# robertknight/ocrs

Measured on AMD Instinct MI355X. Metric: pages/sec end-to-end (1024x1024), higher is better.
Workload: dtype f32

## Files before the change

include/ocrs_amd.h:

```cpp
#ifndef OCRS_AMD_H
#define OCRS_AMD_H

#include <stddef.h>
#include <stdint.h>

#if defined(__GNUC__)
#define OCRS_API __attribute__((visibility("default")))
#else
#define OCRS_API
#endif

#ifdef __cplusplus
extern "C" {
#endif

typedef enum ocrs_status {
    OCRS_OK = 0,
    OCRS_ERR_INVALID_ARGUMENT = 1,
    OCRS_ERR_MODEL_NOT_LOADED = 2,
    OCRS_ERR_MODEL_DIMS = 3,
    OCRS_ERR_RUN_FAILED = 4,
    OCRS_ERR_WRONG_OUTPUT = 5,
    OCRS_ERR_IMAGE_SOURCE = 6,
    OCRS_ERR_DEVICE = 7,
    OCRS_ERR_IO = 8,
    OCRS_ERR_CAPACITY = 9
} ocrs_status;

OCRS_API const char* ocrs_last_error(void);

#define OCRS_ABI_VERSION 6u
OCRS_API uint32_t ocrs_abi_version(void);

OCRS_API void ocrs_buffer_free(void* p);

OCRS_API ocrs_status ocrs_device_count(int* n);
OCRS_API ocrs_status ocrs_set_device(int device);
OCRS_API ocrs_status ocrs_get_device(int* device);

OCRS_API ocrs_status ocrs_ctc_beam_search(const float* logp, int t, int c, uint32_t width, int impl, uint32_t** labels,
                                          uint32_t** positions, size_t* n);
OCRS_API ocrs_status ocrs_ctc_beam_search_scored(const float* logp, int t, int c, uint32_t width, int impl, uint32_t** labels,
                                                 uint32_t** positions, size_t* n, double* score, float** step_logp);

OCRS_API ocrs_status ocrs_gru_tile_plan(const int32_t* lengths_desc, size_t n_lines, int hidden, int32_t* n_clusters, int32_t* waves,
                                        int16_t* tiles);

OCRS_API ocrs_status ocrs_coalescer_selftest(int n_threads, int requests_per_thread, int max_active, int max_pages,
                                             long window_us, int fail_every, uint64_t out[5]);

OCRS_API ocrs_status ocrs_set_option(const char* name, long value);
OCRS_API ocrs_status ocrs_option_name(int index, const char** name);

OCRS_API ocrs_status ocrs_device_pool_stats(int device, uint64_t out[12]);
OCRS_API ocrs_status ocrs_device_pool_configure(int device, uint64_t device_cached_cap_bytes, uint64_t pinned_cached_cap_bytes);
OCRS_API ocrs_status ocrs_device_pool_trim(int device);

typedef enum { OCRS_ISOLATION_AUTO = 0, OCRS_ISOLATION_NONE = 1 } ocrs_isolation;
OCRS_API ocrs_status ocrs_device_set_isolation(int device, ocrs_isolation policy);
OCRS_API ocrs_status ocrs_device_isolation(int device, int out[3]);

typedef struct ocrs_model ocrs_model;

OCRS_API ocrs_status ocrs_model_load_file(const char* path, ocrs_model** out);
OCRS_API ocrs_status ocrs_model_load_bytes(const void* data, size_t len, ocrs_model** out);
OCRS_API ocrs_status ocrs_model_load_file_on_device(const char* path, int device, ocrs_model** out);
OCRS_API ocrs_status ocrs_model_load_bytes_on_device(const void* data, size_t len, int device, ocrs_model** out);
OCRS_API ocrs_status ocrs_model_device(const ocrs_model* m, int* device);

typedef int (*ocrs_model_run_fn)(void* user, const float* input, const int64_t in_shape[4], float** output,
                                 int64_t out_shape[4], int* out_ndim);
OCRS_API ocrs_status ocrs_model_from_callback(const int64_t input_shape[4],
                                     ocrs_model_run_fn run, void* user, ocrs_model** out);

OCRS_API ocrs_status ocrs_model_input_shape(const ocrs_model* m, int64_t dims[4], uint8_t is_fixed[4]);

typedef struct ocrs_run_options {
    int timing;
} ocrs_run_options;

OCRS_API ocrs_status ocrs_model_run(const ocrs_model* m, const float* input, const int64_t in_shape[4],
                           const ocrs_run_options* opts, float** output, int64_t out_shape[4], int* out_ndim);

OCRS_API ocrs_status ocrs_model_flops(const ocrs_model* m, const int64_t in_shape[4], double* flops);

OCRS_API void ocrs_model_free(ocrs_model* m);

typedef struct ocrs_engine ocrs_engine;
typedef struct ocrs_page ocrs_page;

typedef enum ocrs_numerics { OCRS_NUMERICS_EXACT = 0, OCRS_NUMERICS_RELAXED = 1, OCRS_NUMERICS_REDUCED = 2 } ocrs_numerics;

typedef enum ocrs_decode_method {
    OCRS_DECODE_GREEDY = 0,
    OCRS_DECODE_BEAM_SEARCH = 1
} ocrs_decode_method;

typedef struct ocrs_engine_params {
    const ocrs_model* detection_model;
    const ocrs_model* recognition_model;
    int debug;
    ocrs_decode_method decode_method;
    uint32_t beam_width;
    const char* alphabet;
    const char* allowed_chars;
    ocrs_numerics numerics;
    int coalesce;
    int coalesce_pages;
    int coalesce_window_us;
    int layout_threads;
    int64_t rec_max_pixels;
} ocrs_engine_params;

OCRS_API ocrs_status ocrs_engine_new(const ocrs_engine_params* params, ocrs_engine** out);
OCRS_API void ocrs_engine_free(ocrs_engine* e);
OCRS_API ocrs_status ocrs_engine_device(const ocrs_engine* e, int* device);
OCRS_API ocrs_status ocrs_engine_set_option(ocrs_engine* e, const char* name, long value);
OCRS_API ocrs_status ocrs_engine_get_option(const ocrs_engine* e, const char* name, long* value);

typedef enum ocrs_dim_order { OCRS_HWC = 0, OCRS_CHW = 1 } ocrs_dim_order;
typedef enum ocrs_pixel_type { OCRS_U8 = 0, OCRS_F32 = 1 } ocrs_pixel_type;

OCRS_API ocrs_status ocrs_image_source_check_bytes(size_t len, uint32_t width, uint32_t height, uint32_t* channels);

OCRS_API ocrs_status ocrs_engine_prepare_input(const ocrs_engine* e, const void* pixels, ocrs_pixel_type type,
                                      ocrs_dim_order order, int height, int width, int channels,
                                      ocrs_page** out);
OCRS_API ocrs_status ocrs_engine_prepare_input_batch(const ocrs_engine* e, const void* const* pixels, size_t n,
                                                     ocrs_pixel_type type, ocrs_dim_order order, int height, int width,
// ... 244 lines not shown
```

ocrs_amd/_lib.py:

```python
import ctypes as C
import os

_HERE = os.path.dirname(os.path.abspath(__file__))
LIB_PATH = os.environ.get("OCRS_AMD_LIB") or os.path.join(_HERE, "libocrs_amd.so")

OCRS_OK = 0
STATUS_NAMES = {
    0: "OK", 1: "INVALID_ARGUMENT", 2: "MODEL_NOT_LOADED", 3: "MODEL_DIMS", 4: "RUN_FAILED", 5: "WRONG_OUTPUT",
    6: "IMAGE_SOURCE", 7: "DEVICE", 8: "IO", 9: "CAPACITY",
}

RUN_FN = C.CFUNCTYPE(C.c_int, C.c_void_p, C.POINTER(C.c_float), C.POINTER(C.c_int64), C.POINTER(C.POINTER(C.c_float)),
                     C.POINTER(C.c_int64), C.POINTER(C.c_int))


class EngineParams(C.Structure):
    _fields_ = [("detection_model", C.c_void_p), ("recognition_model", C.c_void_p), ("debug", C.c_int),
                ("decode_method", C.c_int), ("beam_width", C.c_uint32), ("alphabet", C.c_char_p),
                ("allowed_chars", C.c_char_p), ("numerics", C.c_int), ("coalesce", C.c_int), ("coalesce_pages", C.c_int),
                ("coalesce_window_us", C.c_int), ("layout_threads", C.c_int), ("rec_max_pixels", C.c_int64)]


class GroupParams(C.Structure):
    _fields_ = [("detection_model", C.c_void_p), ("detection_model_len", C.c_size_t), ("recognition_model", C.c_void_p),
                ("recognition_model_len", C.c_size_t), ("devices", C.POINTER(C.c_int)), ("n_devices", C.c_size_t),
                ("debug", C.c_int), ("decode_method", C.c_int), ("beam_width", C.c_uint32), ("alphabet", C.c_char_p),
                ("allowed_chars", C.c_char_p), ("gather", C.c_int), ("numerics", C.c_int), ("coalesce", C.c_int),
                ("coalesce_pages", C.c_int), ("coalesce_window_us", C.c_int), ("layout_threads", C.c_int), ("rec_max_pixels", C.c_int64),
                ("min_block", C.c_int), ("shared_block", C.c_int)]


class RunOptions(C.Structure):
    _fields_ = [("timing", C.c_int)]


class TextCharC(C.Structure):
    _fields_ = [("ch", C.c_uint32), ("top", C.c_int32), ("left", C.c_int32), ("bottom", C.c_int32),
                ("right", C.c_int32)]


class OcrsError(RuntimeError):
    def __init__(self, status, message):
        super().__init__(message)
        self.status = status
        self.status_name = STATUS_NAMES.get(status, str(status))


DECLARED_SYMBOLS = [
    "ocrs_last_error", "ocrs_buffer_free", "ocrs_device_count", "ocrs_set_device", "ocrs_set_option", "ocrs_ctc_beam_search", "ocrs_model_load_file",
    "ocrs_model_load_bytes", "ocrs_model_from_callback", "ocrs_model_input_shape", "ocrs_model_run",
    "ocrs_model_flops", "ocrs_model_free", "ocrs_engine_new", "ocrs_engine_free", "ocrs_image_source_check_bytes",
    "ocrs_engine_prepare_input", "ocrs_engine_prepare_input_device", "ocrs_page_free", "ocrs_page_dims",
    "ocrs_page_image", "ocrs_engine_detect_words", "ocrs_engine_detect_words_batch",
    "ocrs_engine_detect_text_pixels", "ocrs_engine_detection_threshold", "ocrs_engine_find_text_lines",
    "ocrs_engine_find_text_lines_batch",
    "ocrs_engine_recognize_text", "ocrs_engine_recognize_text_batch", "ocrs_engine_recognize_tokens",
    "ocrs_engine_prepare_recognition_input", "ocrs_text_item_rotated_rect", "ocrs_rotated_rect_corners", "ocrs_engine_get_text", "ocrs_device_malloc", "ocrs_device_free",
    "ocrs_device_upload", "ocrs_device_synchronize", "ocrs_device_measure_peaks", "ocrs_engine_enable_timing", "ocrs_stage_count",
    "ocrs_stage_name", "ocrs_engine_stage_times", "ocrs_kernel_class_count", "ocrs_kernel_class_name",
    "ocrs_engine_kernel_stats", "ocrs_engine_set_kernel_timing_mask", "ocrs_gru_tile_plan", "ocrs_host_malloc", "ocrs_host_free", "ocrs_engine_prepare_input_batch",
    "ocrs_get_device", "ocrs_model_load_file_on_device", "ocrs_model_load_bytes_on_device", "ocrs_model_device", "ocrs_engine_device",
    "ocrs_engine_group_new", "ocrs_engine_group_free", "ocrs_engine_group_size", "ocrs_engine_group_member", "ocrs_group_deal",
    "ocrs_group_prepare_input_batch", "ocrs_group_prepare_input_device_batch", "ocrs_group_detect_words_batch",
    "ocrs_group_recognize_text_batch", "ocrs_group_gather", "ocrs_group_final_gather", "ocrs_group_worker_threads", "ocrs_group_last_gather", "ocrs_device_malloc_on", "ocrs_engine_coalesce_stats", "ocrs_coalescer_selftest", "ocrs_engine_kernel_mfma_flops", "ocrs_engine_prepare_input_jpeg", "ocrs_jpeg_decode_rgb", "ocrs_jpeg_info", "ocrs_jpeg_coefficients",
    "ocrs_group_member_stats", "ocrs_numa_parse_cpulist", "ocrs_numa_bind_selftest", "ocrs_engine_recognize_logits", "ocrs_engine_set_option", "ocrs_engine_get_option", "ocrs_option_name", "ocrs_device_pool_stats", "ocrs_device_pool_configure", "ocrs_device_pool_trim",
    "ocrs_device_set_isolation", "ocrs_device_isolation", "ocrs_group_set_replay", "ocrs_abi_version",
    "ocrs_engine_recognize_text_scored", "ocrs_engine_recognize_text_batch_scored", "ocrs_ctc_beam_search_scored",
    "ocrs_engine_run_recognition_ops",
    "ocrs_engine_detect_words_scored", "ocrs_engine_detect_words_batch_scored", "ocrs_group_detect_words_batch_scored",
    "ocrs_engine_find_text_lines_indexed", "ocrs_engine_find_text_lines_batch_indexed",
    "ocrs_detection_tile_plan", "ocrs_engine_detect_words_tiled", "ocrs_engine_detect_words_batch_tiled",
    "ocrs_engine_detect_text_pixels_tiled", "ocrs_group_detect_words_batch_tiled",
    "ocrs_line_frame", "ocrs_line_char_boxes", "ocrs_engine_prepare_recognition_input_rectified",
    "ocrs_engine_recognize_text_rectified", "ocrs_engine_recognize_text_batch_rectified",
    "ocrs_group_recognize_text_batch_rectified", "ocrs_engine_recognize_tokens_rectified",
    "ocrs_engine_rotate_page", "ocrs_engine_rotate_pages", "ocrs_unrotate_rects", "ocrs_unrotate_chars",
    "ocrs_orientation_vote", "ocrs_engine_detect_orientation", "ocrs_engine_page_from_grey",
    "ocrs_engine_resize_page", "ocrs_engine_resize_pages", "ocrs_work_size", "ocrs_rescale_rects",
    "ocrs_engine_detect_words_at", "ocrs_engine_detect_words_batch_at",
    "ocrs_normalize_params_default", "ocrs_normalize_params_check", "ocrs_engine_normalize_page", "ocrs_engine_normalize_pages",
]

ABI_VERSION = 6
TILE_OVERLAP_DEFAULT = 100
RESAMPLE_FILTERS = {"auto": 0, "bilinear": 1, "area": 2}
POLARITIES = {"auto": 0, "keep": 1, "invert": 2}


class NormalizeParams(C.Structure):
    _fields_ = [("tile", C.c_int32), ("polarity", C.c_int32), ("flatten", C.c_int32), ("levels", C.c_int32)]


class NormalizeInfo(C.Structure):
    _fields_ = [("dark", C.c_int32), ("white", C.c_int32), ("lo", C.c_int32), ("hi", C.c_int32), ("vote", C.c_int64),
                ("counted", C.c_uint64)]

    def as_dict(self):
        return {"dark": int(self.dark), "vote": int(self.vote), "white": int(self.white), "lo": int(self.lo), "hi": int(self.hi),
                "counted": int(self.counted)}

_lib = None


def lib():
    global _lib
    if _lib is None:
        if not os.path.exists(LIB_PATH):
            raise OcrsError(7, "libocrs_amd.so is not built: run `python -m ocrs_amd.build` "
                               "(there is no CPU fallback for the HIP engine)")
        L = C.CDLL(LIB_PATH)
        L.ocrs_abi_version.restype = C.c_uint32
        if L.ocrs_abi_version() != ABI_VERSION:
            raise OcrsError(7, "libocrs_amd.so has ABI version %d, this binding was written for %d: rebuild (python -m ocrs_amd.build)"
                            % (L.ocrs_abi_version(), ABI_VERSION))
        L.ocrs_last_error.restype = C.c_char_p
        L.ocrs_engine_detection_threshold.restype = C.c_float
        L.ocrs_engine_detection_threshold.argtypes = [C.c_void_p]
        L.ocrs_stage_name.restype = C.c_char_p
        L.ocrs_kernel_class_name.restype = C.c_char_p
        L.ocrs_buffer_free.argtypes = [C.c_void_p]
        for name in ("ocrs_model_free", "ocrs_engine_free", "ocrs_page_free", "ocrs_engine_group_free"):
            getattr(L, name).argtypes = [C.c_void_p]
            getattr(L, name).restype = None
        _lib = L
    return _lib


def check(status):
    if status != OCRS_OK:
        msg = lib().ocrs_last_error()
        raise OcrsError(status, msg.decode("utf-8", "replace") if msg else STATUS_NAMES.get(status, "error"))


def device_count():
    n = C.c_int(0)
    check(lib().ocrs_device_count(C.byref(n)))
    return n.value


def measure_peaks():
    a, b = C.c_double(0), C.c_double(0)
    check(lib().ocrs_device_measure_peaks(C.byref(a), C.byref(b)))
    return a.value, b.value
# ... 113 lines not shown
```

ocrs_amd/csrc/abi.cpp:

```cpp
#include <cstdio>
#include <fstream>
#include <thread>

#include <atomic>
#include "abi_util.hpp"
#include "coalesce_selftest.hpp"
#include "engine.hpp"
#include "host_pool.hpp"
#include "jpeg.hpp"
#include "kernels.hpp"
#include "page_ops.hpp"

using namespace ocrs;
using namespace ocrs::geom;

using namespace ocrs::abi;

extern "C" {

const char* ocrs_last_error(void) { return last_error().c_str(); }

void ocrs_buffer_free(void* p) { free(p); }

ocrs_status ocrs_device_count(int* n) {
    return guarded([&] {
        int c = 0;
        hipError_t e = hipGetDeviceCount(&c);
        if (e != hipSuccess) c = 0;
        *n = c;
    });
}

ocrs_status ocrs_set_device(int device) {
    return guarded([&] { select_device(device); });
}

ocrs_status ocrs_get_device(int* device) {
    return guarded([&] {
        if (!device) fail(OCRS_ERR_INVALID_ARGUMENT, "null argument");
        *device = default_device();
    });
}

ocrs_status ocrs_gru_tile_plan(const int32_t* lengths_desc, size_t n_lines, int hidden, int32_t* n_clusters, int32_t* waves,
                               int16_t* tiles) {
    return guarded([&] {
        if (!lengths_desc || !n_clusters || !waves || !tiles || n_lines == 0 || n_lines > (size_t)1 << 20)
            fail(OCRS_ERR_INVALID_ARGUMENT, "bad argument");
        for (size_t i = 0; i < n_lines; i++)
            if (lengths_desc[i] < 1 || (i > 0 && lengths_desc[i] > lengths_desc[i - 1]))
                fail(OCRS_ERR_INVALID_ARGUMENT, "lengths must be positive and descending");
        int ncl = 0;
        if (!k::gru_tile_plan(lengths_desc, (int)n_lines, hidden, &ncl, waves, tiles))
            fail(OCRS_ERR_CAPACITY, "no persistent-kernel plan for this shape (the engine then runs the recurrence as one fused launch per time step)");
        *n_clusters = ncl;
    });
}

ocrs_status ocrs_coalescer_selftest(int n_threads, int requests_per_thread, int max_active, int max_pages, long window_us,
                                    int fail_every, uint64_t out[5]) {
    return guarded([&] {
        if (!out || n_threads < 1 || requests_per_thread < 1 || max_pages < 1) fail(OCRS_ERR_INVALID_ARGUMENT, "bad argument");
        coalescer_selftest(n_threads, requests_per_thread, max_active, max_pages, window_us, fail_every, out);
    });
}

namespace {

void beam_search_hook(const float* logp, int t, int c, uint32_t width, int impl, std::vector<uint32_t>* l,
                      std::vector<uint32_t>* p, double* score, std::vector<float>* step_logp) {
    if (impl == 2 && t > 0) {
        DeviceScope bind(-1);
        if (!k::ctc_beam_supported(c, (int)width)) fail(OCRS_ERR_CAPACITY, "beam search on the GPU supports up to 128 classes and width 128");
        Workspace ws;
        std::vector<int32_t> meta(1 + t + 1);
        meta[0] = t;
        for (int i = 0; i <= t; i++) meta[1 + i] = i;
        int32_t* d_meta = ws.alloc_n<int32_t>(meta.size());
        float* d_logp = ws.alloc_n<float>((size_t)t * c);
        ws.upload(d_meta, meta.data(), meta.size() * sizeof(int32_t));
        ws.upload(d_logp, logp, (size_t)t * c * sizeof(float));
        const size_t arena = k::ctc_beam_arena_entries(t, (int)width);
        int2* d_nodes = ws.alloc_n<int2>(arena);
        int2* d_posn = ws.alloc_n<int2>(arena);
        uint32_t* d_ol = ws.alloc_n<uint32_t>(t);
        uint32_t* d_op = ws.alloc_n<uint32_t>(t);
        int32_t* d_cnt = ws.alloc_n<int32_t>(1);
        double* d_score = score ? ws.alloc_n<double>(1) : nullptr;
        float* d_slp = score ? ws.alloc_n<float>(t) : nullptr;
        k::ctc_beam_packed(d_logp, d_meta, d_meta + 1, 1, t, c, (int)width, nullptr, d_nodes, d_posn, d_ol, d_op, d_cnt, ws.s(),
                           d_score, d_slp);
        std::vector<uint32_t> hl(t), hp(t);
        std::vector<float> hs(score ? t : 0);
        int32_t cnt = 0;
        ws.download(hl.data(), d_ol, (size_t)t * 4);
        ws.download(hp.data(), d_op, (size_t)t * 4);
        ws.download(&cnt, d_cnt, 4);
        if (score) {
            ws.download(score, d_score, sizeof(double));
            ws.download(hs.data(), d_slp, (size_t)t * sizeof(float));
        }
        ws.sync();
        OCRS_HIP(hipGetLastError());
        l->assign(hl.begin(), hl.begin() + cnt);
        p->assign(hp.begin(), hp.begin() + cnt);
        if (score) step_logp->assign(hs.begin(), hs.begin() + cnt);
    } else {
        double bs = 0.0;
        const std::vector<CtcStep> st = t == 0 ? std::vector<CtcStep>()
                                              : (impl == 1 ? ctc_beam_search_reference(logp, t, c, c, width, &bs)
                                                           : ctc_beam_search(logp, t, c, c, width, &bs));
        l->resize(st.size()); p->resize(st.size());
        for (size_t i = 0; i < st.size(); i++) { (*l)[i] = st[i].label; (*p)[i] = st[i].pos; }
        if (score) score_line(logp, t, c, c, nullptr, st, &bs, step_logp, score);
    }
}

}

ocrs_status ocrs_ctc_beam_search(const float* logp, int t, int c, uint32_t width, int impl, uint32_t** labels,
                                 uint32_t** positions, size_t* n) {
    return guarded([&] {
        if (!logp || !labels || !positions || !n || t < 0 || c < 1) fail(OCRS_ERR_INVALID_ARGUMENT, "bad argument");
        std::vector<uint32_t> l, p;
        beam_search_hook(logp, t, c, width, impl, &l, &p, nullptr, nullptr);
        *labels = dup_buffer(l);
        *positions = dup_buffer(p);
        *n = l.size();
    });
}

ocrs_status ocrs_ctc_beam_search_scored(const float* logp, int t, int c, uint32_t width, int impl, uint32_t** labels,
                                        uint32_t** positions, size_t* n, double* score, float** step_logp) {
    return guarded([&] {
        if (!logp || !labels || !positions || !n || !score || !step_logp || t < 0 || c < 1)
            fail(OCRS_ERR_INVALID_ARGUMENT, "bad argument");
        std::vector<uint32_t> l, p;
        std::vector<float> s;
// ... 952 lines not shown
```

ocrs_amd/csrc/common.cpp:

```cpp
#include "common.hpp"

#include <chrono>
#include <climits>
#include <cstdint>
#include <cstdlib>
#include <cstring>

#include <algorithm>
#include <atomic>
#include <condition_variable>
#include <deque>
#include <system_error>

namespace ocrs {

static thread_local std::string g_last_error;

void set_last_error(const std::string& msg) { g_last_error = msg; }
const std::string& last_error() { return g_last_error; }

namespace {
std::atomic<int> g_default_device{0};
thread_local DeviceContext* t_ctx = nullptr;
constexpr int kMaxDevices = 64;
// ... 302 lines not shown
    if (mode == MODE_SERIAL) return heavy_stream();
    std::lock_guard<std::mutex> g(lazy_mu_);
    if (!recurrent_) {
        DeviceScope bind(device);
        int least = 0, greatest = 0;
        OCRS_HIP(hipDeviceGetStreamPriorityRange(&least, &greatest));
        OCRS_HIP(hipStreamCreateWithPriority(&recurrent_, hipStreamNonBlocking, greatest));
    }
    return recurrent_;
}

static thread_local int t_lease_depth[kMaxDevices] = {0};

template <class F> void DeviceContext::switch_isolation(F&& change) {
    if (t_lease_depth[device] > 0) fail(OCRS_ERR_INVALID_ARGUMENT, "the isolation regime of device %d cannot change from inside one of its requests", device);
    std::unique_lock<std::mutex> lk(iso_mu_);
    iso_cv_.wait(lk, [&] { return !switching_; });
    const Mode before = mode_locked();
    switching_ = true;
    struct Done { DeviceContext* c; ~Done() { c->switching_ = false; c->iso_cv_.notify_all(); } } done{this};
    const Isolation p0 = policy_;
    const int r0 = relaxed_;
    change();
    if (mode_locked() == before) return;
    const Isolation p1 = policy_;
    const int r1 = relaxed_;
    policy_ = p0; relaxed_ = r0;
    iso_cv_.wait(lk, [&] { return leases_ == 0; });
    {
        DeviceScope bind(device);
        if (hipDeviceSynchronize() != hipSuccess) (void)hipGetLastError();
    }
    policy_ = p1; relaxed_ = r1;
}

DeviceContext::Mode DeviceContext::lease_begin() {
    std::unique_lock<std::mutex> lk(iso_mu_);
    if (t_lease_depth[device] == 0) iso_cv_.wait(lk, [&] { return !switching_; });
    t_lease_depth[device]++;
    leases_++;
    return mode_locked();
}

void DeviceContext::lease_end() {
    std::lock_guard<std::mutex> lk(iso_mu_);
    t_lease_depth[device]--;
    if (--leases_ == 0) iso_cv_.notify_all();
}

void DeviceContext::add_relaxed_engine(int delta) {
    switch_isolation([&] { relaxed_ += delta; });
}

void DeviceContext::set_isolation(Isolation policy) {
    switch_isolation([&] { policy_ = policy; });
}

DeviceContext::Mode DeviceContext::current_mode() {
    std::lock_guard<std::mutex> lk(iso_mu_);
    return mode_locked();
}

int DeviceContext::relaxed_engine_count() {
    std::lock_guard<std::mutex> lk(iso_mu_);
    return relaxed_;
}

int DeviceContext::cu_count() {
    std::lock_guard<std::mutex> g(lazy_mu_);
    if (!cus_) {
        hipDeviceProp_t prop;
        OCRS_HIP(hipGetDeviceProperties(&prop, device));
        cus_ = prop.multiProcessorCount;
    }
    return cus_;
}

namespace {
struct OptDef { const char* name; const char* env; long def; };
const OptDef kOptDefs[OPT_COUNT] = {
    {"gru_mode", "OCRS_GRU_MODE", GRU_PERSISTENT},
    {"gru_gates", "OCRS_GRU_GATES", 1},
    {"gru_local", "OCRS_GRU_LOCAL", 1},
    {"det_fuse", "OCRS_DET_FUSE", 1},
    {"det_stream", "OCRS_DET_STREAM", 1},
    {"det_rows", "OCRS_DET_ROWS", 1},
    {"ccl_quad", "OCRS_CCL_QUAD", 1},
    {"conv12_fuse", "OCRS_CONV12_FUSE", 1},
    {"conv_flat", "OCRS_CONV_FLAT", 1},
    {"beam_gpu", "OCRS_BEAM_GPU", 1},
    {"det_tile_batch", "OCRS_DET_TILE_BATCH", 16},
    {"numerics", nullptr, 0},
    {"coalesce", nullptr, 2},
    {"coalesce_pages", nullptr, 16},
    {"coalesce_window_us", nullptr, 300},
    {"layout_threads", nullptr, 0},
    {"rec_max_pixels", nullptr, 0},
};
struct OptRange { long lo, hi; long also[4]; };
const OptRange kOptRanges[OPT_COUNT] = {
    {0, 1, {}}, {0, 1, {}}, {0, 1, {}}, {0, 2, {}}, {0, 1, {8, 14, 32}}, {0, 1, {8, 14, 20, 32}}, {0, 1, {}}, {0, 1, {}}, {0, 1, {}}, {0, 1, {}},
    {1, 1024, {}},
    {0, 2, {}}, {0, 64, {}}, {1, 4096, {}}, {0, 10000000, {}}, {0, 4096, {}}, {0, INT64_MAX, {}},
};
bool in_range(int i, long v) {
    const OptRange& r = kOptRanges[i];
    if (v >= r.lo && v <= r.hi) return true;
    for (long a : r.also) if (a && v == a) return true;
    return false;
}
const char* const kRetired[] = {"det_heavy", "det_tail", "gru_waves", "gru_background", "gru_scatter", "gru_gates_pack", "conv_occupancy",
                                "gx_heavy", "gemm_nfast", "conv_a_lds", "gru_heavy", "heavy_priority", "det_mfma"};
std::atomic<long> g_opts[OPT_COUNT];
std::once_flag g_opts_once;
void init_options() {
    for (int i = 0; i < OPT_COUNT; i++) {
        const char* e = kOptDefs[i].env ? getenv(kOptDefs[i].env) : nullptr;
        const long v = e && *e ? strtol(e, nullptr, 10) : kOptDefs[i].def;
        g_opts[i].store(in_range(i, v) ? v : kOptDefs[i].def);
    }
}
int find_option(const char* name, int count = OPT_PUBLIC_COUNT) {
    for (int i = 0; i < count; i++)
        if (name && i != OPT_NUMERICS && strcmp(name, kOptDefs[i].name) == 0) return i;
    return -1;
}
thread_local const Tuning* t_tuning = nullptr;
}

TuningScope::TuningScope(const Tuning* t) : prev_(t_tuning) { t_tuning = t; }
TuningScope::~TuningScope() { t_tuning = prev_; }
const Tuning* current_tuning() { return t_tuning; }

long option_long(Option o) {
    if (t_tuning) return __atomic_load_n(&t_tuning->v[o], __ATOMIC_RELAXED);
    std::call_once(g_opts_once, init_options);
    return g_opts[o].load(std::memory_order_relaxed);
}
int option(Option o) { return (int)option_long(o); }

Tuning default_tuning() {
    std::call_once(g_opts_once, init_options);
    Tuning t;
    for (int i = 0; i < OPT_COUNT; i++) t.v[i] = g_opts[i].load(std::memory_order_relaxed);
    return t;
}

const char* option_name(int i) { return i >= 0 && i < OPT_PUBLIC_COUNT ? kOptDefs[i].name : nullptr; }

int set_option(const char* name, long value) {
    std::call_once(g_opts_once, init_options);
    const int i = find_option(name);
    if (i < 0) {
        for (const char* r : kRetired) if (name && strcmp(name, r) == 0) return 0;
        return 1;
    }
    if (!in_range(i, value)) return 2;
    g_opts[i].store(value);
    return 0;
}

int set_option(Tuning& t, const char* name, long value) {
    const int i = find_option(name, OPT_COUNT);
    if (i < 0) return 1;
    if (!in_range(i, value)) return 2;
    __atomic_store_n(&t.v[i], value, __ATOMIC_RELAXED);
    return 0;
}

bool get_option(const Tuning& t, const char* name, long* value) {
    const int i = name && strcmp(name, "numerics") == 0 ? (int)OPT_NUMERICS : find_option(name, OPT_COUNT);
    if (i < 0) return false;
    *value = __atomic_load_n(&t.v[i], __ATOMIC_RELAXED);
    return true;
}

StreamLease::StreamLease(bool high_priority) : ctx_(&ctx()), high_(high_priority) {
    high_ = true;
    mode_ = ctx_->lease_begin();
    try {
        if (mode_ == DeviceContext::MODE_SERIAL) {
            s_ = ctx_->heavy_stream();
            shared_ = true;
            OCRS_HIP(hipEventCreateWithFlags(&done_, hipEventBlockingSync | hipEventDisableTiming));
// ... 114 lines not shown
```

ocrs_amd/csrc/common.hpp:

```cpp
#pragma once
#include <atomic>
#include <hip/hip_runtime.h>

#include <cstdarg>
#include <cstdint>
#include <cstdio>
#include <cstdlib>
#include <chrono>
#include <condition_variable>
#include <cstring>
#include <map>
#include <mutex>
#include <stdexcept>
#include <string>
#include <thread>
#include <vector>

#include "../../include/ocrs_amd.h"

namespace ocrs {

struct Error : std::runtime_error {
    ocrs_status status;
    Error(ocrs_status s, const std::string& msg) : std::runtime_error(msg), status(s) {}
// ... 33 lines not shown

  private:
    uint64_t cap_locked();
    const int device_;
    std::mutex mu_;
    std::multimap<size_t, void*> free_;
    std::map<void*, size_t> live_;
    uint64_t cached_ = 0, live_bytes_ = 0, peak_live_ = 0, cap_ = 0, allocs_ = 0;
    std::atomic<uint64_t> frees_{0};
};

class HostPool {
  public:
    void* alloc(size_t bytes);
    void release(void* p);
    void set_cap(uint64_t bytes);
    PoolStats stats();

  private:
    std::mutex mu_;
    std::multimap<size_t, void*> free_;
    std::map<void*, size_t> live_;
    uint64_t cached_ = 0, live_bytes_ = 0, peak_live_ = 0, cap_ = uint64_t(1) << 30, allocs_ = 0;
    std::atomic<uint64_t> frees_{0};
};

struct DeviceContext {
    const int device;
    DevicePool pool;
    HostPool host_pool;
    std::mutex heavy_phase, rec_phase;
    hipStream_t heavy_stream();
    hipStream_t recurrent_stream(int mode = 0);
    enum Isolation { ISO_AUTO = 0, ISO_NONE = 1 };
    enum Mode { MODE_FREE = 0, MODE_SERIAL = 1 };
    Mode lease_begin();
    void lease_end();
    void add_relaxed_engine(int delta);
    void set_isolation(Isolation policy);
    Mode current_mode();
    int relaxed_engine_count();
    int cu_count();
    std::vector<struct DevBuf> heavy_arena;
    std::mutex stream_mu;
    std::vector<std::pair<hipStream_t, hipEvent_t>> streams;

    explicit DeviceContext(int d) : device(d), pool(d) {}

  private:
    Mode mode_locked() const { return policy_ == ISO_NONE || relaxed_ <= 0 ? MODE_FREE : MODE_SERIAL; }
    template <class F> void switch_isolation(F&& change);
    std::mutex lazy_mu_;
    hipStream_t heavy_ = nullptr, recurrent_ = nullptr;
    int cus_ = 0;
    std::mutex iso_mu_;
    std::condition_variable iso_cv_;
    int leases_ = 0, relaxed_ = 0;
    bool switching_ = false;
    Isolation policy_ = ISO_AUTO;
    friend class StreamLease;
};

DeviceContext& device_context(int device);
int default_device();
void select_device(int device);
DeviceContext& ctx();

class DeviceScope {
  public:
    explicit DeviceScope(int device);
    ~DeviceScope();
    DeviceScope(const DeviceScope&) = delete;
    DeviceScope& operator=(const DeviceScope&) = delete;

  private:
    DeviceContext* prev_;
    int restore_ = -1;
};

inline DevicePool& pool() { return ctx().pool; }
inline HostPool& host_pool() { return ctx().host_pool; }
inline hipStream_t heavy_stream() { return ctx().heavy_stream(); }

enum Option { OPT_GRU_MODE = 0, OPT_GRU_GATES, OPT_GRU_LOCAL, OPT_DET_FUSE, OPT_DET_STREAM, OPT_DET_ROWS, OPT_CCL_QUAD,
              OPT_CONV12_FUSE, OPT_CONV_FLAT, OPT_BEAM_GPU, OPT_DET_TILE_BATCH, OPT_PUBLIC_COUNT,
              OPT_NUMERICS = OPT_PUBLIC_COUNT,
              OPT_COALESCE, OPT_COALESCE_PAGES, OPT_COALESCE_WINDOW_US,
              OPT_LAYOUT_THREADS, OPT_REC_MAX_PIXELS,
              OPT_COUNT };
struct Tuning { long v[OPT_COUNT]; };
Tuning default_tuning();
int set_option(const char* name, long value);
int set_option(Tuning& t, const char* name, long value);
bool get_option(const Tuning& t, const char* name, long* value);
const char* option_name(int i);
class TuningScope {
  public:
    explicit TuningScope(const Tuning* t);
    ~TuningScope();
    TuningScope(const TuningScope&) = delete;
    TuningScope& operator=(const TuningScope&) = delete;
  private:
    const Tuning* prev_;
};
const Tuning* current_tuning();
enum { GRU_PERSISTENT = 0, GRU_STEP = 1 };
int option(Option o);

inline void allow_dynamic_lds(const void* kernel, std::atomic<uint64_t>& done) {
    int dev = 0;
    (void)hipGetDevice(&dev);
    const uint64_t bit = 1ull << (dev & 63);
    if (done.load(std::memory_order_relaxed) & bit) return;
    (void)hipFuncSetAttribute(kernel, hipFuncAttributeMaxDynamicSharedMemorySize, 160 * 1024);
    done.fetch_or(bit, std::memory_order_relaxed);
}
long option_long(Option o);
inline int gru_mode() { return option(OPT_GRU_MODE); }

struct DevBuf {
    void* p = nullptr;
    size_t bytes = 0;
    DevicePool* owner = nullptr;
    DevBuf() = default;
    explicit DevBuf(size_t n) : bytes(n), owner(n ? &pool() : nullptr) { p = n ? owner->alloc(n) : nullptr; }
    DevBuf(const DevBuf&) = delete;
    DevBuf& operator=(const DevBuf&) = delete;
    DevBuf(DevBuf&& o) noexcept : p(o.p), bytes(o.bytes), owner(o.owner) { o.p = nullptr; o.bytes = 0; o.owner = nullptr; }
    DevBuf& operator=(DevBuf&& o) noexcept {
        if (this != &o) { reset(); p = o.p; bytes = o.bytes; owner = o.owner; o.p = nullptr; o.bytes = 0; o.owner = nullptr; }
        return *this;
    }
    ~DevBuf() { reset(); }
    void reset() { if (p && owner) owner->release(p); p = nullptr; bytes = 0; owner = nullptr; }
    int device() const { return owner ? owner->device() : -1; }
    template <class T> T* as() const { return static_cast<T*>(p); }
};

struct PinnedBuf {
    void* p = nullptr;
    size_t bytes = 0;
    PinnedBuf() = default;
    explicit PinnedBuf(size_t n) : bytes(n) { if (n) OCRS_HIP(hipHostMalloc(&p, n, hipHostMallocPortable)); }
    PinnedBuf(const PinnedBuf&) = delete;
    PinnedBuf& operator=(const PinnedBuf&) = delete;
    ~PinnedBuf() { if (p) (void)hipHostFree(p); }
    template <class T> T* as() const { return static_cast<T*>(p); }
};

class StreamLease {
  public:
    explicit StreamLease(bool high_priority = false);
    ~StreamLease();
    hipStream_t get() const { return s_; }
    hipError_t wait_done() const noexcept {
        hipError_t e = hipEventRecord(done_, s_);
        if (e != hipSuccess) return e;
        for (int i = 0;; i++) {
            e = hipEventQuery(done_);
            if (e != hipErrorNotReady) return e;
            if (i < 64) std::this_thread::yield();
            else std::this_thread::sleep_for(std::chrono::microseconds(i < 256 ? 20 : 100));
        }
    }
    void sync() const { OCRS_HIP(wait_done()); }
    hipError_t sync_noexcept() const noexcept { return wait_done(); }
    DeviceContext::Mode mode() const { return mode_; }
// ... 133 lines not shown
```

ocrs_amd/csrc/kernels.hpp:

```cpp
#pragma once
#include <vector>
#include <hip/hip_runtime.h>

#include <cstdint>

namespace ocrs {
namespace jpeg { struct Coefficients; }
namespace k {

void prepare_image(const void* d_pixels, bool is_u8, bool chans_last, int h, int w, int chans, float* d_out,
                   hipStream_t s);
void resize_pages_to_model(const float* const* d_src_ptrs, int n, int sh, int sw, int vh, int vw, float* d_dst,
                           int dh, int dw, hipStream_t s);
bool resize_threshold(const float* d_prob, int n, int mh, int mw, int sh, int sw, float thr, uint8_t* d_mask,
                      float* d_map, int h, int w, hipStream_t s, int32_t* d_labels = nullptr, int32_t* d_zero_a = nullptr,
                      int32_t* d_zero_b = nullptr);
void threshold_only(const float* d_prob, float thr, uint8_t* d_mask, int64_t count, hipStream_t s);

struct CclBuffers {
    int32_t* labels;
    int32_t* row_counts;
    int32_t* row_offsets;
    int32_t* n_roots;
    int32_t* roots;
    int32_t* lengths;
    int32_t* offsets;
    int32_t* overflow;
    uint32_t* pts;
    uint32_t* tmp;
    uint8_t* keep;
    float* rects;
    uint8_t* valid;
    uint32_t* score_pixels;
    unsigned long long* score_sums;
};
void ccl_label(const uint8_t* d_mask, int n, int h, int w, const CclBuffers& b, int max_comp, hipStream_t s, bool prepared = false);
void contour_rects(const uint8_t* d_mask, int n, int h, int w, const CclBuffers& b, int max_comp, int64_t arena,
                   float expand, float min_area, float eps, hipStream_t s, bool prepared = false);

void component_scores(const uint8_t* d_mask, const float* d_map, int n, int h, int w, const CclBuffers& b, int max_comp,
                      hipStream_t s);

struct TileDesc {
    const float* page;
    uint8_t* mask;
    float* map;
    int32_t h, w;
    int32_t oy, ox;
    int32_t y0, y1, x0, x1;
};
void gather_tiles(const TileDesc* d_tiles, int n_tiles, float* d_dst, int mh, int mw, hipStream_t s);
void stitch_threshold(const TileDesc* d_tiles, int n_tiles, const float* d_prob, int mh, int mw, float thr, hipStream_t s);

struct GemmDesc {
    const float* A; int lda;
    const float* B; int ldb;
    const float* bias;
    float* C; int ldc;
    int M, N, K;
    int relu;
    int im2col; int H, W, Cin;
    int convt; int Cout;
    int batch; int64_t strideA, strideB, strideBias, strideC;
    int nfast = 0, nx = 0, ny = 0;
    const uint16_t* Bsplit = nullptr; int64_t strideBsplit = 0;
};
void gemm(const GemmDesc& d, hipStream_t s);
void conv_direct(const float* x, int n, int h, int w, int cin, const float* wt, const float* bias, int kh, int kw,
                 int cout, int relu, float* y, hipStream_t s);
void dwconv3x3(const float* x, int n, int h, int w, int c, const float* wt, const float* bias, int relu, float* y,
               hipStream_t s);
bool dwpw_fused_supported(int cin, int cout);
void dwpw_fused(const float* x, int n, int h, int w, int cin, const float* wdw, const float* bdw, int relu_dw, int cout,
                const float* wpw, const float* bpw, int relu_pw, float* y, hipStream_t s);
bool dwconv3x3_cat(const float* skip, int n, int h, int w, int cs, const float* up, int uh, int uw, int cu, const float* wt,
                   const float* bias, int relu, float* y, hipStream_t s);
struct DoubleConvArgs {
    const float* skip;
    const float* x1;
    const float *wt, *bt;
    const float *wd1, *bd1;
    const float *wp1, *bp1;
    const float *wd2, *bd2;
    const float *wp2, *bp2;
    const float *wf, *bf;
    float* y;
    float* ypool;
    int n, h, w, h1, w1;
    int relu_d1, relu_p1, relu_d2, relu_p2, sigmoid;
    int tiles_x, tiles_y;
    const float* tape = nullptr;
    int tape_len = 0;
    const float* rtape = nullptr;
    int rtape_len = 0;
};
struct StreamWeights {
    const float *wt, *bt, *wd1, *bd1, *wp1, *bp1, *wd2, *bd2, *wp2, *bp2, *wf, *bf;
};
bool double_conv_fused(const DoubleConvArgs& a, int cs, int cx, int cmid, int cout, bool pool, bool final_conv,
                       bool launch, hipStream_t s, bool* on_mfma = nullptr, int* path = nullptr);
bool double_conv_stream(const DoubleConvArgs& a, int cs, int cx, int cmid, int cout, bool pool, bool final_conv, bool launch, hipStream_t s,
                        const StreamWeights* hw = nullptr, std::vector<float>* tape_out = nullptr, int* tape_len = nullptr);
bool double_conv_rows(const DoubleConvArgs& a, int cs, int cx, int cmid, int cout, bool pool, bool final_conv, bool launch, hipStream_t s,
                      const StreamWeights* hw = nullptr, std::vector<float>* tape_out = nullptr, int* tape_len = nullptr);
bool double_conv_rows_takes(const DoubleConvArgs& a, int cx);
void maxpool(const float* x, int n, int h, int w, int c, int kh, int kw, float* y, hipStream_t s);
void avgpool(const float* x, int n, int h, int w, int c, int kh, int kw, float* y, hipStream_t s);
void padcat(const float* skip, int n, int sh, int sw, int cs, const float* x, int h, int w, int cx, float* y,
            hipStream_t s);
void sigmoid(const float* x, float* y, int64_t count, hipStream_t s);
void conv1x1_cout1(const float* x, int64_t pixels, int cin, const float* wt, const float* bias, int relu, int do_sigmoid,
                   float* y, hipStream_t s);
void to_seq(const float* x, int n, int w, int c, float* y, hipStream_t s);
void gru_gates(const float* gx, const float* gh, float* h, float* y, int T, int N, int H, int step, hipStream_t s);
bool log_softmax_argmax(const float* logits, int64_t rows, int c, const uint8_t* d_excluded ,
                        float* logp, int32_t* labels, hipStream_t s, float* maxlp = nullptr);
void to_seq_packed(const float* x, int n, int T, int c, const int32_t* d_pos, const int32_t* d_off, float* y,
                   hipStream_t s);
void gru_gates_packed(const float* gx, const float* gh, float* h, float* y, const int32_t* d_Tm, const int32_t* d_off,
                      int64_t R, int Mcap, int active, int H, int step, hipStream_t s);
bool gru_step_fused(const float* gx, const float* wh, const float* bh, const float* hT_in, float* hT_out, float* y,
                    const int32_t* d_Tm, const int32_t* d_off, int64_t R, int Mcap, int active, int H, int step,
                    hipStream_t s);
size_t gru_persistent_sync_words(int M);
size_t gru_persistent_exchange_bytes(const int32_t* h_Tm, int M, int H);
bool gru_persistent_supported(const int32_t* h_Tm, int M, int Tmax, int64_t R, int H);
bool gru_tile_plan(const int32_t* h_Tm, int M, int H, int* ncl, int* waves, int16_t* tiles );
hipError_t gru_persistent_prepare(float* hx, const int32_t* h_Tm, int M, int H, hipStream_t s);
bool gru_persistent(const float* gx, const float* wh, const float* bh, float* y, float* hx, const int32_t* d_Tm, const int32_t* d_off,
                    const int32_t* h_Tm, int64_t R, int M, int Tmax, int H, uint32_t* d_sync, hipStream_t s);
bool gru_general_tile_plan(const int32_t* h_Tm, int M, int Tmax, int H, int cap, int* ncl, int16_t* tiles , int kernel );
size_t gru_split_exchange_bytes(const int32_t* h_Tm, int M, int H, int np);
bool gru_split_supported(const int32_t* h_Tm, int M, int Tmax, int64_t R, int H, int np);
hipError_t gru_split_prepare(uint16_t* hx, const int32_t* h_Tm, int M, int H, int np, hipStream_t s);
bool gru_persistent_split(const float* gx, const float* wh, const float* bh, float* y, uint16_t* hx, const int32_t* d_Tm, const int32_t* d_off,
                          const int32_t* h_Tm, int64_t R, int M, int Tmax, int H, int np, uint32_t* d_sync, hipStream_t s);
void ctc_collapse_packed(const int32_t* labels, const int32_t* d_Tm, const int32_t* d_off, int M, int Tmax,
                         uint32_t* out_labels, uint32_t* out_pos, int32_t* out_count, hipStream_t s);
void ctc_collapse_scored_packed(const int32_t* labels, const float* maxlp, const int32_t* d_Tm, const int32_t* d_off, int M,
                                int Tmax, uint32_t* out_labels, uint32_t* out_pos, float* out_logp, int32_t* out_count,
                                double* out_score, hipStream_t s);
void argmax_rows(const float* x, int64_t rows, int c, const uint8_t* d_excluded, int32_t* labels, hipStream_t s);
bool ctc_beam_supported(int C, int width);
size_t ctc_beam_arena_entries(int Tmax, int width);
bool ctc_beam_packed(const float* logp, const int32_t* d_Tm, const int32_t* d_off, int M, int Tmax, int C, int width,
                     const uint8_t* d_excluded, int2* d_nodes, int2* d_posn, uint32_t* out_labels, uint32_t* out_pos,
                     int32_t* out_count, hipStream_t s, double* out_score = nullptr, float* out_logp = nullptr);
void ctc_collapse(const int32_t* labels, int T, int N, uint32_t* out_labels, uint32_t* out_pos, int32_t* out_count,
                  hipStream_t s);

struct RaggedView {
    int G;
    int H;
    const int32_t* W;
    const int32_t* n;
    const int64_t* poff;
    const int32_t* toff128;
    const int32_t* toff256;
    const int32_t* loff;
    int ntiles128, ntiles256;
    const int32_t* toff2d;
    int ntiles2d, tw;
    const int32_t* toff2d_flat;
    const int32_t* toff2d_flat2;
    int ntiles2d_flat, ntiles2d_flat2;
    const int32_t* toff2d_gap;
    int ntiles2d_gap;
    int64_t max_tile_px_;
    int min_w;
    int64_t pixels;
    int max_w;
};
void conv1_relu_pool_ragged(const float* x, const RaggedView& in, const float* wt, const float* bias, int cout,
                            float* y, const RaggedView& out, hipStream_t s);
void pool_ragged(const float* x, const RaggedView& in, int c, int kh, int kw, bool avg, float* y, const RaggedView& out,
                 hipStream_t s);
void to_seq_packed_ragged(const float* x, const RaggedView& in, int c, const int32_t* d_pos, const int32_t* d_off,
                          float* y, hipStream_t s);
void avgpool_to_seq_ragged(const float* x, const RaggedView& in, const RaggedView& seq, int c, const int32_t* d_pos,
                           const int32_t* d_off, float* y, hipStream_t s);
bool conv12_fused_ragged(const float* x, const RaggedView& in0, const RaggedView& mid, const float* w1, const float* b1,
                         int c1, const float* w2, const float* b2, int c2, float* y, const RaggedView& out, hipStream_t s,
                         const uint16_t* w2split = nullptr);
void conv12_split_weights(const float* w2_host , std::vector<uint16_t>* out);
bool conv3x3_ragged(const float* x, const RaggedView& rv, int cin, const float* wt, const float* bias, int cout, int relu,
                    int ph, int pw, float* y, const RaggedView& out, hipStream_t s, const uint16_t* wsplit = nullptr);
void split_weights(const float* w_host, int K, int N, int ldw, std::vector<uint16_t>* out);

struct LineDesc {
    int32_t page;
    int32_t poly_off;
    int32_t poly_n;
    int32_t top, left, bh, bw;
    int32_t resized_w;
    int32_t out_w;
    int64_t out_off;
};
void crop_lines(const float* const* d_pages, const int32_t* d_page_hw , const LineDesc* d_lines,
                const int32_t* d_poly , int n_lines, int out_h, float* d_out, hipStream_t s);

struct RectLineDesc {
    int32_t page;
    int32_t mode;
    int32_t range_off;
    int32_t range_n;
    int32_t resized_w;
    int32_t out_w;
    int64_t out_off;
    float x0, ax, bx, y0, ay, by;
};
void rectify_lines(const float* const* d_pages, const int32_t* d_page_hw , const RectLineDesc* d_lines,
                   const int32_t* d_ranges, int n_lines, int max_out_w, int out_h, float* d_out, hipStream_t s);

// ... 63 lines not shown
```

ocrs_amd/csrc/kernels_gru.hip:

```cpp
#include <algorithm>
#include <cstdlib>
#include <map>
#include <mutex>
#include <vector>

#include "common.hpp"
#include "kernels.hpp"
#include "spec_math.hpp"

namespace ocrs {
namespace k {

typedef float f32x4 __attribute__((ext_vector_type(4)));
typedef unsigned u32x2 __attribute__((ext_vector_type(2)));

namespace {

constexpr int kMaxSlots = 128;

struct GruParams {
    const float* gx;
    const float* wh;
    const float* bh;
    float* y;
    float* hx;
    const int32_t* Tm;
    const int32_t* off;
    uint32_t* sync;
    uint32_t* place;
    int64_t R;
    int M, ncl, Tmax;
    int prio;
    int allow_local;
    int16_t tiles[kMaxSlots * 4];
    int32_t tbase[kMaxSlots * 4];
    int TB;
    uint32_t spin_limit;
};

typedef unsigned u32x4 __attribute__((ext_vector_type(4)));
constexpr int kAuxSc1 = 16;
__device__ __forceinline__ f32x4 load_bypass(__amdgpu_buffer_rsrc_t y, uint32_t byte_off) {
    return __builtin_bit_cast(f32x4, __builtin_amdgcn_raw_buffer_load_b128(y, (int)byte_off, 0, kAuxSc1));
}
__device__ __forceinline__ void store_through(__amdgpu_buffer_rsrc_t y, uint32_t byte_off, f32x4 v) {
    __builtin_amdgcn_raw_buffer_store_b128(__builtin_bit_cast(u32x4, v), y, (int)byte_off, 0, kAuxSc1);
}
__device__ __forceinline__ void store_local(__amdgpu_buffer_rsrc_t y, uint32_t byte_off, f32x4 v) {
    __builtin_amdgcn_raw_buffer_store_b128(__builtin_bit_cast(u32x4, v), y, (int)byte_off, 0, 0);
}
typedef __attribute__((address_space(1))) uint32_t gu32;

__device__ __forceinline__ void transpose4(const f32x4& in, float* out) {
    const unsigned v0 = __float_as_uint(in[0]), v1 = __float_as_uint(in[1]);
    const unsigned v2 = __float_as_uint(in[2]), v3 = __float_as_uint(in[3]);
    const u32x2 p01 = __builtin_amdgcn_permlane16_swap(v0, v1, false, false);
    const u32x2 p23 = __builtin_amdgcn_permlane16_swap(v2, v3, false, false);
    const u32x2 q02 = __builtin_amdgcn_permlane32_swap(p01[0], p23[0], false, false);
    const u32x2 q13 = __builtin_amdgcn_permlane32_swap(p01[1], p23[1], false, false);
    out[0] = __uint_as_float(q02[0]);
    out[1] = __uint_as_float(q13[0]);
    out[2] = __uint_as_float(q02[1]);
    out[3] = __uint_as_float(q13[1]);
}

constexpr unsigned kUnwritten = 0xFFFFFFFFu;

template <int H>
struct Loaded {
    f32x4 h[H / 16];
    f32x4 hp;
    f32x4 gr, gz, gn;
    uint32_t out_off;
    uint32_t hx_off;
    uint32_t prev_off;
    bool has_prev;
    bool active;
};

template <int H>
__device__ __forceinline__ void issue_meta(const GruParams& p, int dir, int ub, int tile, int tbase, int tm, const int* off_l, int s,
                                           int i16, int kq, Loaded<H>& L) {
    const int m = tile * 16 + i16;
    L.active = tm > s;
    const int t = dir ? tm - 1 - s : s;
    const int64_t row = L.active ? (int64_t)off_l[t] + m : 0;
    L.out_off = (uint32_t)((row * 2 * H + dir * H + ub * 16 + kq * 4) * sizeof(float));
    const f32x4 zero = {0.0f, 0.0f, 0.0f, 0.0f};
    L.gr = L.gz = L.gn = zero;
    L.has_prev = L.active && s > 0;
    L.prev_off = 0;
    const uint32_t blk = (uint32_t)(dir * p.TB + tbase + s);
    L.hx_off = (blk * (H / 16) + ub) * 1024u + i16 * 64u + kq * 16u;
    if (L.active) {
        const float* g = p.gx + ((int64_t)dir * p.R + row) * 3 * H + ub * 16 + kq * 4;
        L.gr = *reinterpret_cast<const f32x4*>(g);
        L.gz = *reinterpret_cast<const f32x4*>(g + H);
        L.gn = *reinterpret_cast<const f32x4*>(g + 2 * H);
        if (s > 0) L.prev_off = (blk - 1u) * (H / 16) * 1024u + i16 * 64u;
    }
}

template <int H>
__device__ __forceinline__ void issue_state(__amdgpu_buffer_rsrc_t y, int ub, int kq, Loaded<H>& L) {
    constexpr uint32_t kPiece = 1024u;
    if (L.has_prev) {
#pragma unroll
        for (int j = 0; j < H / 16; j++) L.h[j] = load_bypass(y, L.prev_off + j * kPiece + kq * 16);
        L.hp = load_bypass(y, L.prev_off + ub * kPiece + kq * 16);
    } else {
        const f32x4 zero = {0.0f, 0.0f, 0.0f, 0.0f};
#pragma unroll
        for (int j = 0; j < H / 16; j++) L.h[j] = zero;
        L.hp = zero;
    }
}

template <int H>
__device__ __forceinline__ bool state_ready(const Loaded<H>& L) {
    unsigned mx = 0;
#pragma unroll
    for (int j = 0; j < H / 16; j++)
#pragma unroll
        for (int e = 0; e < 4; e++) mx = max(mx, __float_as_uint(L.h[j][e]));
#pragma unroll
    for (int e = 0; e < 4; e++) mx = max(mx, __float_as_uint(L.hp[e]));
    return !__any(mx == kUnwritten);
}

template <int H>
__device__ __forceinline__ bool await_state(const GruParams& p, __amdgpu_buffer_rsrc_t y, int ub, int kq, Loaded<H>& L) {
    for (uint32_t spins = 0; !state_ready<H>(L); spins++) {
        __builtin_amdgcn_s_sleep(2);
        if (spins >= 4u) {
            const uint32_t n = spins < 36u ? (spins >> 2) : 9u;
            for (uint32_t z = 0; z < n; z++) __builtin_amdgcn_s_sleep(16);
        }
        if ((spins & 255u) == 255u) {
            gu32* err = (gu32*)p.sync;
            const uint32_t e = __builtin_amdgcn_readfirstlane(__hip_atomic_load(err, __ATOMIC_RELAXED, __HIP_MEMORY_SCOPE_AGENT));
            if (e != 0 || spins >= p.spin_limit) {
                __hip_atomic_store(err, 1u, __ATOMIC_RELAXED, __HIP_MEMORY_SCOPE_AGENT);
                return false;
            }
        }
        issue_state<H>(y, ub, kq, L);
    }
    return true;
}

struct GateAcc { f32x4 r, z, n; };

template <int H>
__device__ __forceinline__ GateAcc mfma_chain(int lane, const float (&w)[H / 4], const float* lds_w, const f32x4& br,
                                              const f32x4& bz, const f32x4& bn) {
    f32x4 acc_r = br, acc_z = bz, acc_n = bn;
    const f32x4* ap = reinterpret_cast<const f32x4*>(lds_w) + lane;
    f32x4 ar = ap[0], az = ap[(H / 16) * 64], an = ap[2 * (H / 16) * 64];
#pragma unroll
    for (int blk = 0; blk < H / 16; blk++) {
        f32x4 nr = ar, nz = az, nn = an;
        if (blk + 1 < H / 16) {
            nr = ap[(blk + 1) * 64];
            nz = ap[((H / 16) + blk + 1) * 64];
            nn = ap[(2 * (H / 16) + blk + 1) * 64];
        }
#pragma unroll
        for (int e = 0; e < 4; e++) {
            const float b = w[4 * blk + e];
            acc_r = __builtin_amdgcn_mfma_f32_16x16x4f32(ar[e], b, acc_r, 0, 0, 0);
            acc_z = __builtin_amdgcn_mfma_f32_16x16x4f32(az[e], b, acc_z, 0, 0, 0);
            acc_n = __builtin_amdgcn_mfma_f32_16x16x4f32(an[e], b, acc_n, 0, 0, 0);
        }
        ar = nr; az = nz; an = nn;
    }
    return GateAcc{acc_r, acc_z, acc_n};
}

__device__ __forceinline__ float expf_sl(float x0) {
    float x = x0 > 88.0f ? 88.0f : x0;
    x = x < -87.0f ? -87.0f : x;
    const float kf = rintf(x * 1.44269504088896341f);
    float r = fmaf(kf, -0.693145751953125f, x);
    r = fmaf(kf, -1.42860682030941723212e-6f, r);
    float q = 1.98412698412698413e-4f;
    q = fmaf(q, r, 1.38888888888888894e-3f);
    q = fmaf(q, r, 8.33333333333333322e-3f);
    q = fmaf(q, r, 4.16666666666666644e-2f);
    q = fmaf(q, r, 1.66666666666666657e-1f);
    q = fmaf(q, r, 0.5f);
    q = fmaf(q, r, 1.0f);
    q = fmaf(q, r, 1.0f);
    const float v = __int_as_float(__float_as_int(q) + (((int)kf) << 23));
    return x0 != x0 ? x0 : v;
}
template <bool FAST>
__device__ __forceinline__ float sigmoid_g(float x) {
    if (FAST) return __builtin_amdgcn_rcpf(1.0f + __builtin_amdgcn_exp2f(x * -1.44269504088896341f));
    return 1.0f / (1.0f + expf_sl(-x));
}
template <bool FAST>
__device__ __forceinline__ float tanh_g(float x) {
    if (FAST) {
        const float t = __builtin_amdgcn_exp2f((x > 40.0f ? 40.0f : x) * 2.88539008177792682f);
        return (t - 1.0f) * __builtin_amdgcn_rcpf(t + 1.0f);
    }
    const float t = expf_sl(2.0f * x);
    return (t - 1.0f) / (t + 1.0f);
}

template <int H, bool FAST>
__device__ __forceinline__ f32x4 epilogue_store(__amdgpu_buffer_rsrc_t y, const GateAcc& a, const f32x4& gr, const f32x4& gz,
                                                const f32x4& gn, const f32x4& hp, uint32_t out_off, bool store, bool local) {
    f32x4 hn;
#pragma unroll
    for (int r = 0; r < 4; r++) {
        const float rg = sigmoid_g<FAST>(gr[r] + a.r[r]);
        const float zg = sigmoid_g<FAST>(gz[r] + a.z[r]);
        const float ng = tanh_g<FAST>(fmaf(rg, a.n[r], gn[r]));
        const float hv = fmaf(zg, hp[r] - ng, ng);
        hn[r] = __float_as_uint(hv) == kUnwritten ? __uint_as_float(0x7FC00000u) : hv;
    }
    const uint32_t o = store ? out_off : 0xFFFFFFF0u;
    if (local) store_local(y, o, hn);
    else store_through(y, o, hn);
    return hn;
}

template <int H, bool FAST>
__global__ void __launch_bounds__(256)
gru_persistent_kernel(GruParams p) {
    extern __shared__ __attribute__((aligned(16))) float lds_w[];
    constexpr int UB = H / 16;
    constexpr int WV = 4;
    constexpr bool EARLY = true;
    const int b = blockIdx.x;
    const int q = b >> 3;
    const int ub = q % UB;
    const int cid = (q / UB) * 8 + (b & 7);
    if (cid >= 2 * p.ncl) return;
    const int dir = cid & 1, cl = cid >> 1;
    const int tid = threadIdx.x;
    const int lane = tid & 63;
    const int wave = __builtin_amdgcn_readfirstlane(tid >> 6);
    const int i16 = lane & 15, kq = lane >> 4;
    uint32_t xcc;
    asm volatile("s_getreg_b32 %0, hwreg(HW_REG_XCC_ID, 0, 4)" : "=s"(xcc));
    if (tid == 0) __hip_atomic_store((gu32*)p.place + cid * UB + ub, xcc + 1u, __ATOMIC_RELAXED, __HIP_MEMORY_SCOPE_AGENT);
    const float* __restrict__ whd = p.wh + (int64_t)dir * H * 3 * H;
    const float* __restrict__ bhd = p.bh + (int64_t)dir * 3 * H;
    const int j0 = ub * 16;
    for (int i = tid; i < H * 12; i += 64 * WV) {
        const int k = i / 12, qq = i - k * 12;
        const int g = qq >> 2, c4 = (qq & 3) * 4;
        const float4 v = *reinterpret_cast<const float4*>(whd + (int64_t)k * 3 * H + g * H + j0 + c4);
        const int blk = k >> 4, e = (k >> 2) & 3, kk = k & 3;
        float* dst = &lds_w[(((g * (H / 16) + blk) * 64) + kk * 16 + c4) * 4 + e];
        dst[0] = v.x; dst[4] = v.y; dst[8] = v.z; dst[12] = v.w;
    }
    int* off_l = reinterpret_cast<int*>(lds_w + H * 48);
    for (int i = tid; i <= p.Tmax; i += 64 * WV) off_l[i] = p.off[i];
    const f32x4 br = *reinterpret_cast<const f32x4*>(bhd + j0 + kq * 4);
    const f32x4 bz = *reinterpret_cast<const f32x4*>(bhd + H + j0 + kq * 4);
    const f32x4 bn = *reinterpret_cast<const f32x4*>(bhd + 2 * H + j0 + kq * 4);
    const int slot = cl * WV + wave;
    const int t0 = p.tiles[slot * 4 + 0], t1 = p.tiles[slot * 4 + 1], t2 = p.tiles[slot * 4 + 2], t3 = p.tiles[slot * 4 + 3];
    auto tile_of = [&](int i) { return i == 0 ? t0 : i == 1 ? t1 : i == 2 ? t2 : t3; };
    int tmr[4], tT[4];
#pragma unroll
    for (int i = 0; i < 4; i++) {
        const int m = tile_of(i) * 16 + i16;
        tmr[i] = (tile_of(i) >= 0 && m < p.M) ? p.Tm[m] : 0;
        tT[i] = __builtin_amdgcn_readfirstlane(tmr[i]);
    }
    auto sel = [](const int (&a)[4], int i) { return i == 0 ? a[0] : i == 1 ? a[1] : i == 2 ? a[2] : i == 3 ? a[3] : 0; };
    __syncthreads();
    if (p.prio >= 3) __builtin_amdgcn_s_setprio(3);
    else if (p.prio == 2) __builtin_amdgcn_s_setprio(2);
    else if (p.prio == 1) __builtin_amdgcn_s_setprio(1);
    if (tT[0] <= 0) return;
    bool local;
    {
        const gu32* pl = (const gu32*)p.place + cid * UB;
        uint32_t v = xcc + 1u;
        for (uint32_t spins = 0;; spins++) {
            if (lane < UB) v = __hip_atomic_load(pl + lane, __ATOMIC_RELAXED, __HIP_MEMORY_SCOPE_AGENT);
            if (!__any(v == 0u)) break;
            __builtin_amdgcn_s_sleep(8);
            if (spins >= p.spin_limit) {
                __hip_atomic_store((gu32*)p.sync, 1u, __ATOMIC_RELAXED, __HIP_MEMORY_SCOPE_AGENT);
                return;
            }
        }
        local = !__any(v != xcc + 1u) && p.allow_local;
    }
    const __amdgpu_buffer_rsrc_t yb = __builtin_amdgcn_make_buffer_rsrc(p.y, 0, (int)(uint32_t)(p.R * 2 * H * sizeof(float)), 0x00020000);
    const __amdgpu_buffer_rsrc_t hxb = __builtin_amdgcn_make_buffer_rsrc(p.hx, 0, (int)((uint32_t)p.TB * 2u * (H / 16) * 1024u), 0x00020000);
    const int tb0 = p.tbase[slot * 4 + 0], tb1 = p.tbase[slot * 4 + 1], tb2 = p.tbase[slot * 4 + 2], tb3 = p.tbase[slot * 4 + 3];
    auto tbase_of = [&](int i) { return i == 0 ? tb0 : i == 1 ? tb1 : i == 2 ? tb2 : tb3; };
    int s = 0, i = 0;
#ifdef OCRS_GRU_PROBE
    uint64_t pr_tr = 0, pr_mma = 0, pr_gate = 0, pr_wait = 0, pr_items = 0, pr_t0 = __builtin_readcyclecounter();
#endif
    Loaded<H> bufA, bufB;
    issue_meta<H>(p, dir, ub, tile_of(0), tbase_of(0), tmr[0], off_l, 0, i16, kq, bufA);
    issue_state<H>(hxb, ub, kq, bufA);
    auto item = [&](Loaded<H>& cur, Loaded<H>& nxt) -> int {
        int ns = s, ni = i + 1;
        if (sel(tT, ni) <= s) { ns = s + 1; ni = 0; }
        const bool have_next = sel(tT, ni) > ns;
        const bool early = EARLY && have_next && ni != i;
#ifdef OCRS_GRU_PROBE
        const uint64_t pt0 = __builtin_readcyclecounter();
#endif
        float w[H / 4];
#pragma unroll
        for (int j = 0; j < H / 16; j++) transpose4(cur.h[j], &w[4 * j]);
        if (have_next) issue_meta<H>(p, dir, ub, tile_of(ni), tbase_of(ni), sel(tmr, ni), off_l, ns, i16, kq, nxt);
        if (early) issue_state<H>(hxb, ub, kq, nxt);
#ifdef OCRS_GRU_PROBE
        asm volatile("" :: "v"(w[0]), "v"(w[H / 4 - 1]));
        const uint64_t pt1 = __builtin_readcyclecounter();
#endif
        const GateAcc acc = mfma_chain<H>(lane, w, lds_w, br, bz, bn);
#ifdef OCRS_GRU_PROBE
        asm volatile("" :: "v"(acc.r), "v"(acc.z), "v"(acc.n));
        const uint64_t pt2 = __builtin_readcyclecounter();
#endif
        const f32x4 hn = epilogue_store<H, FAST>(hxb, acc, cur.gr, cur.gz, cur.gn, cur.hp, cur.hx_off, cur.active, local);
        store_local(yb, cur.active ? cur.out_off : 0xFFFFFFF0u, hn);
#ifdef OCRS_GRU_PROBE
        const uint64_t pt3 = __builtin_readcyclecounter();
        pr_tr += pt1 - pt0; pr_mma += pt2 - pt1; pr_gate += pt3 - pt2; pr_items++;
#endif
        if (!have_next) return 0;
        if (!early) issue_state<H>(hxb, ub, kq, nxt);
        if (!await_state<H>(p, hxb, ub, kq, nxt)) return -1;
#ifdef OCRS_GRU_PROBE
        pr_wait += __builtin_readcyclecounter() - pt3;
#endif
        s = ns;
        i = ni;
        return 1;
    };
    for (;;) {
        if (item(bufA, bufB) <= 0) break;
        if (item(bufB, bufA) <= 0) break;
    }
#ifdef OCRS_GRU_PROBE
    if (cid == 0 && ub == 0 && lane == 0)
        printf("probe fp32 wave %d local %d tiles %d: items %llu, cycles per item %llu = transposes + issue %llu | chain %llu | gates + stores %llu | wait %llu\n", wave, (int)local,
               (t0 >= 0) + (t1 >= 0) + (t2 >= 0) + (t3 >= 0), (unsigned long long)pr_items, (unsigned long long)((__builtin_readcyclecounter() - pr_t0) / pr_items),
               (unsigned long long)(pr_tr / pr_items), (unsigned long long)(pr_mma / pr_items), (unsigned long long)(pr_gate / pr_items), (unsigned long long)(pr_wait / pr_items));
#endif
}



template <int H>
__device__ __forceinline__ f32x4 gate_chain(int lane, const float (&w)[H / 4], const float* lds_w, int g, const f32x4& bias) {
    f32x4 acc = bias;
    const f32x4* ap = reinterpret_cast<const f32x4*>(lds_w) + g * (H / 16) * 64 + lane;
    f32x4 a = ap[0];
#pragma unroll
    for (int blk = 0; blk < H / 16; blk++) {
        f32x4 na = a;
        if (blk + 1 < H / 16) na = ap[(blk + 1) * 64];
#pragma unroll
        for (int e = 0; e < 4; e++) acc = __builtin_amdgcn_mfma_f32_16x16x4f32(a[e], w[4 * blk + e], acc, 0, 0, 0);
        a = na;
    }
    return acc;
}

template <int H, bool FAST>
__global__ void __launch_bounds__(256)
gru_gates_kernel(GruParams p) {
    extern __shared__ __attribute__((aligned(16))) float lds_w[];
    asm volatile("v_accvgpr_write_b32 a200, 0" ::: "a200");
    constexpr int UB = H / 16;
    const int b = blockIdx.x;
    const int q = b >> 3;
    const int ub = q % UB;
    const int cid = (q / UB) * 8 + (b & 7);
    if (cid >= 2 * p.ncl) return;
    const int dir = cid & 1, tile = cid >> 1;
    const int tid = threadIdx.x;
    const int lane = tid & 63;
    const int wave = __builtin_amdgcn_readfirstlane(tid >> 6);
    const int i16 = lane & 15, kq = lane >> 4;
    uint32_t xcc;
    asm volatile("s_getreg_b32 %0, hwreg(HW_REG_XCC_ID, 0, 4)" : "=s"(xcc));
    if (tid == 0) __hip_atomic_store((gu32*)p.place + cid * UB + ub, xcc + 1u, __ATOMIC_RELAXED, __HIP_MEMORY_SCOPE_AGENT);
    const float* __restrict__ whd = p.wh + (int64_t)dir * H * 3 * H;
    const float* __restrict__ bhd = p.bh + (int64_t)dir * 3 * H;
    const int j0 = ub * 16;
    for (int i = tid; i < H * 12; i += 256) {
        const int k = i / 12, qq = i - k * 12;
        const int g = qq >> 2, c4 = (qq & 3) * 4;
        const float4 v = *reinterpret_cast<const float4*>(whd + (int64_t)k * 3 * H + g * H + j0 + c4);
        const int blk = k >> 4, e = (k >> 2) & 3, kk = k & 3;
        float* dst = &lds_w[(((g * (H / 16) + blk) * 64) + kk * 16 + c4) * 4 + e];
        dst[0] = v.x; dst[4] = v.y; dst[8] = v.z; dst[12] = v.w;
    }
    int* off_l = reinterpret_cast<int*>(lds_w + H * 48);
    for (int i = tid; i <= p.Tmax; i += 256) off_l[i] = p.off[i];
    f32x4* xch = reinterpret_cast<f32x4*>(lds_w + H * 48 + (((p.Tmax + 1) + 3) & ~3));
    int* abort_w = reinterpret_cast<int*>(xch + 3 * 64);
    if (tid == 0) *abort_w = 0;
    const int m = tile * 16 + i16;
    const int tm = m < p.M ? p.Tm[m] : 0;
    const int T = __builtin_amdgcn_readfirstlane(tm);
    __syncthreads();
    if (p.prio >= 3) __builtin_amdgcn_s_setprio(3);
    else if (p.prio == 2) __builtin_amdgcn_s_setprio(2);
    else if (p.prio == 1) __builtin_amdgcn_s_setprio(1);
    if (T <= 0) return;
    bool local;
    {
        const gu32* pl = (const gu32*)p.place + cid * UB;
        uint32_t v = xcc + 1u;
        for (uint32_t spins = 0;; spins++) {
            if (lane < UB) v = __hip_atomic_load(pl + lane, __ATOMIC_RELAXED, __HIP_MEMORY_SCOPE_AGENT);
            if (!__any(v == 0u)) break;
            __builtin_amdgcn_s_sleep(8);
            if (spins >= p.spin_limit) {
                __hip_atomic_store((gu32*)p.sync, 2u, __ATOMIC_RELAXED, __HIP_MEMORY_SCOPE_AGENT);
                *abort_w = 1;
                break;
            }
        }
        local = !__any(v != xcc + 1u) && p.allow_local;
    }
    const __amdgpu_buffer_rsrc_t yb = __builtin_amdgcn_make_buffer_rsrc(p.y, 0, (int)(uint32_t)(p.R * 2 * H * sizeof(float)), 0x00020000);
    const __amdgpu_buffer_rsrc_t hxb = __builtin_amdgcn_make_buffer_rsrc(p.hx, 0, (int)((uint32_t)p.TB * 2u * (H / 16) * 1024u), 0x00020000);
    const uint32_t blk0 = (uint32_t)(dir * p.TB + p.tbase[tile]);
    if (wave < 3) {
        const f32x4 bias = *reinterpret_cast<const f32x4*>(bhd + wave * H + j0 + kq * 4);
        Loaded<H> L;
        const f32x4 zero = {0.0f, 0.0f, 0.0f, 0.0f};
        L.gr = L.gz = L.gn = zero;
        L.out_off = 0;
        for (int s = 0; s < T; s++) {
            L.active = tm > s;
            L.has_prev = L.active && s > 0;
            L.hp = zero;
#pragma unroll
            for (int j = 0; j < H / 16; j++) L.h[j] = zero;
            L.prev_off = L.has_prev ? (blk0 + s - 1u) * (H / 16) * 1024u + i16 * 64u : 0u;
            issue_state<H>(hxb, ub, kq, L);
            if (!await_state<H>(p, hxb, ub, kq, L)) *abort_w = 1;
            float w[H / 4];
#pragma unroll
            for (int j = 0; j < H / 16; j++)
#pragma unroll
                for (int e = 0; e < 4; e++) w[4 * j + e] = L.h[j][e];
            xch[wave * 64 + lane] = gate_chain<H>(lane, w, lds_w, wave, bias);
            __syncthreads();
            if (*abort_w) return;
        }
    } else {
        f32x4 hp = {0.0f, 0.0f, 0.0f, 0.0f};
        f32x4 gr, gz, gn, ngr, ngz, ngn;
        uint32_t out_off, nout_off;
        bool active, nactive;
        auto fetch = [&](int s, f32x4& r_, f32x4& z_, f32x4& n_, uint32_t& o_, bool& a_) {
            a_ = tm > s;
            const int t = dir ? tm - 1 - s : s;
            const int64_t row = a_ ? (int64_t)off_l[t] + m : 0;
            o_ = (uint32_t)((row * 2 * H + dir * H + ub * 16 + kq * 4) * sizeof(float));
            const f32x4 zero = {0.0f, 0.0f, 0.0f, 0.0f};
            r_ = z_ = n_ = zero;
            if (a_) {
                const float* g = p.gx + ((int64_t)dir * p.R + row) * 3 * H + ub * 16 + kq * 4;
                r_ = *reinterpret_cast<const f32x4*>(g);
                z_ = *reinterpret_cast<const f32x4*>(g + H);
                n_ = *reinterpret_cast<const f32x4*>(g + 2 * H);
            }
        };
        fetch(0, gr, gz, gn, out_off, active);
        for (int s = 0; s < T; s++) {
            if (s + 1 < T) fetch(s + 1, ngr, ngz, ngn, nout_off, nactive);
            __syncthreads();
            if (*abort_w) return;
            GateAcc a;
            a.r = xch[lane]; a.z = xch[64 + lane]; a.n = xch[128 + lane];
            f32x4 hn;
#pragma unroll
            for (int r = 0; r < 4; r++) {
                const float rg = sigmoid_g<FAST>(gr[r] + a.r[r]);
                const float zg = sigmoid_g<FAST>(gz[r] + a.z[r]);
                const float ng = tanh_g<FAST>(fmaf(rg, a.n[r], gn[r]));
                const float hv = fmaf(zg, hp[r] - ng, ng);
                hn[r] = __float_as_uint(hv) == kUnwritten ? __uint_as_float(0x7FC00000u) : hv;
            }
            const uint32_t o = active ? ((blk0 + s) * (H / 16) + ub) * 1024u + i16 * 64u + kq * 16u : 0xFFFFFFF0u;
            float t[4];
            transpose4(hn, t);
            const f32x4 ht = {t[0], t[1], t[2], t[3]};
            if (local) store_local(hxb, o, ht);
            else store_through(hxb, o, ht);
            store_local(yb, active ? out_off : 0xFFFFFFF0u, hn);
            if (active) hp = hn;
            gr = ngr; gz = ngz; gn = ngn; out_off = nout_off; active = nactive;
        }
    }
}


}

constexpr int kMaxGrid = 4096;
static size_t gru_gates_lds_bytes(int H, int Tmax) {
    return (size_t)H * 48 * sizeof(float) + (size_t)(((Tmax + 1) + 3) & ~3) * sizeof(int) + 3 * 64 * 16 + 16;
}
static size_t gru_general_lds_bytes(int H, int Tmax) { return (size_t)H * 48 * sizeof(float) + ((size_t)Tmax + 1) * sizeof(int); }
size_t gru_persistent_sync_words(int) { return kMaxGrid + 1; }

static int64_t gru_tile_blocks(const int32_t* h_Tm, int M) {
    int64_t tb = 0;
    for (int m = 0; m < M; m += 16) tb += h_Tm[m];
    return tb;
}
size_t gru_persistent_exchange_bytes(const int32_t* h_Tm, int M, int H) { return (size_t)2 * (size_t)gru_tile_blocks(h_Tm, M) * 16 * H * sizeof(float); }

hipError_t gru_persistent_prepare(float* hx, const int32_t* h_Tm, int M, int H, hipStream_t s) {
    return M > 0 ? hipMemsetAsync(hx, 0xFF, gru_persistent_exchange_bytes(h_Tm, M, H), s) : hipSuccess;
}

static int gru_resident_capacity(int H, bool gates, size_t lds) {
    static std::mutex mu;
    static std::map<int, int> cache;
    int dev = 0;
    if (hipGetDevice(&dev) != hipSuccess) return 0;
    const int key = dev * 8 + (gates ? 4 : 0) + (H == 256 ? 2 : H == 128 ? 1 : 0);
    {
        std::lock_guard<std::mutex> g(mu);
        auto it = cache.find(key);
        if (it != cache.end()) return it->second;
    }
    hipDeviceProp_t prop;
    if (hipGetDeviceProperties(&prop, dev) != hipSuccess) return 0;
    int per_cu = 0;
    hipError_t e;
    if (gates) {
        e = H == 256 ? hipOccupancyMaxActiveBlocksPerMultiprocessor(&per_cu, gru_gates_kernel<256, false>, 256, lds)
          : H == 128 ? hipOccupancyMaxActiveBlocksPerMultiprocessor(&per_cu, gru_gates_kernel<128, false>, 256, lds)
                     : hipOccupancyMaxActiveBlocksPerMultiprocessor(&per_cu, gru_gates_kernel<64, false>, 256, lds);
    } else {
        e = H == 256 ? hipOccupancyMaxActiveBlocksPerMultiprocessor(&per_cu, gru_persistent_kernel<256, false>, 256, lds)
          : H == 128 ? hipOccupancyMaxActiveBlocksPerMultiprocessor(&per_cu, gru_persistent_kernel<128, false>, 256, lds)
                     : hipOccupancyMaxActiveBlocksPerMultiprocessor(&per_cu, gru_persistent_kernel<64, false>, 256, lds);
    }
    if (e != hipSuccess) { (void)hipGetLastError(); per_cu = 0; }
    const int cap = prop.multiProcessorCount * (per_cu > 0 ? 1 : 0);
    std::lock_guard<std::mutex> g(mu);
    cache[key] = cap;
    return cap;
}

// ... 6 lines not shown
    if (max_blocks < 8 * UB) return false;
    int max_ncl = max_blocks / UB / 2;
    if (ntiles > 16 * max_ncl) max_ncl *= 2;
    if (ntiles > 16 * max_ncl || 4 * max_ncl > kMaxSlots) return false;
    *ncl = (ntiles + 3) / 4 < max_ncl ? (ntiles + 3) / 4 : max_ncl;
    return gru_general_lds_bytes(H, Tmax) <= 64 * 1024;
}

static const int kRoundCost[3][5] = {{0, 63, 101, 150, 200}, {0, 54, 91, 128, 170}, {0, 44, 68, 99, 135}};
static void gru_assign_tiles(const int32_t* h_Tm, int M, int ncl, int16_t* tiles, int kernel = 0) {
    const int ntiles = (M + 15) / 16, nslots = 4 * ncl;
    const int* round = kRoundCost[kernel >= 0 && kernel < 3 ? kernel : 0];
    for (int i = 0; i < nslots * 4; i++) tiles[i] = -1;
    std::vector<int> cnt(nslots, 0);
    auto cost = [&](int slot, int extra_len) {
        int64_t tot = 0;
        int len[5], n = cnt[slot];
        for (int i = 0; i < n; i++) len[i] = h_Tm[tiles[slot * 4 + i] * 16];
        if (extra_len > 0) len[n++] = extra_len;
        for (int i = n - 1, below = 0; i >= 0; i--) {
            tot += (int64_t)(len[i] - below) * round[i + 1];
            below = len[i];
        }
        return tot;
    };
    for (int k = 0; k < ntiles; k++) {
        const int len = h_Tm[k * 16];
        int best = -1;
        int64_t best_cost = 0;
        for (int sl = 0; sl < nslots; sl++) {
            if (cnt[sl] >= 4) continue;
            const int64_t cs = cost(sl, len);
            if (best < 0 || cs < best_cost) { best = sl; best_cost = cs; }
        }
        tiles[best * 4 + cnt[best]++] = (int16_t)k;
    }
}

bool gru_tile_plan(const int32_t* h_Tm, int M, int H, int* ncl, int* waves, int16_t* tiles ) {
    for (int i = 0; i < kMaxSlots * 4; i++) tiles[i] = -1;
    *waves = 4;
    if (M <= 0 || !gru_plan(M, h_Tm[0], H, ncl, 256)) return false;
    gru_assign_tiles(h_Tm, M, *ncl, tiles);
    return true;
}

bool gru_general_tile_plan(const int32_t* h_Tm, int M, int Tmax, int H, int cap, int* ncl, int16_t* tiles, int kernel) {
    if (M <= 0 || !gru_plan(M, Tmax, H, ncl, cap)) return false;
    if (tiles) gru_assign_tiles(h_Tm, M, *ncl, tiles, kernel);
    return true;
}

bool gru_persistent_supported(const int32_t* h_Tm, int M, int Tmax, int64_t R, int H) {
    int ncl;
    if (H != 256 && H != 128 && H != 64) return false;
    return M > 0 && (uint64_t)R * 2 * H * sizeof(float) < (uint64_t(1) << 32) && (uint64_t)gru_persistent_exchange_bytes(h_Tm, M, H) < (uint64_t(1) << 32) &&
           gru_plan(M, Tmax, H, &ncl, gru_resident_capacity(H, false, gru_general_lds_bytes(H, Tmax)));
}

static bool gru_gates_plan(int M, int Tmax, int H, int* ncl) {
    if (H != 256 && H != 128 && H != 64) return false;
    if (gru_gates_lds_bytes(H, Tmax) > 64 * 1024) return false;
    const int ntiles = (M + 15) / 16, UB = H / 16;
    int cap = gru_resident_capacity(H, true, gru_gates_lds_bytes(H, Tmax));
    cap = cap > 256 ? 256 : cap;
    cap -= cap % (8 * UB);
    if (cap < 8 * UB || ntiles > cap / UB / 2) return false;
    *ncl = ntiles;
    return true;
}

template <int H>
static void launch_gates(bool fast, dim3 grid, size_t lds, hipStream_t s, const GruParams& g) {
    if (fast) hipLaunchKernelGGL((gru_gates_kernel<H, true>), grid, dim3(256), lds, s, g);
    else hipLaunchKernelGGL((gru_gates_kernel<H, false>), grid, dim3(256), lds, s, g);
}
template <int H>
static void launch_general(bool fast, dim3 grid, size_t lds, hipStream_t s, const GruParams& g) {
    if (fast) hipLaunchKernelGGL((gru_persistent_kernel<H, true>), grid, dim3(256), lds, s, g);
    else hipLaunchKernelGGL((gru_persistent_kernel<H, false>), grid, dim3(256), lds, s, g);
}

bool gru_persistent(const float* gx, const float* wh, const float* bh, float* y, float* hx, const int32_t* d_Tm, const int32_t* d_off,
                    const int32_t* h_Tm, int64_t R, int M, int Tmax, int H, uint32_t* d_sync, hipStream_t s) {
    if (M <= 0) return true;
    if (!hx || !gru_persistent_supported(h_Tm, M, Tmax, R, H)) return false;
    const bool fast = option(OPT_NUMERICS) != 0;
    GruParams p{};
    p.gx = gx; p.wh = wh; p.bh = bh; p.y = y; p.hx = hx; p.Tm = d_Tm; p.off = d_off;
    std::vector<int32_t> base((M + 15) / 16 + 1, 0);
    for (size_t k = 0; k + 1 < base.size(); k++) base[k + 1] = base[k] + h_Tm[k * 16];
    p.TB = base.back();
    p.place = d_sync;
    p.sync = d_sync + kMaxGrid;
    p.R = R; p.M = M; p.Tmax = Tmax;
    p.prio = 3;
    p.spin_limit = 1u << 21;
    p.allow_local = option(OPT_GRU_LOCAL) != 0;
    const int UB = H / 16;
    if (option(OPT_GRU_GATES) && gru_gates_plan(M, Tmax, H, &p.ncl)) {
        for (int k = 0; k < p.ncl; k++) p.tbase[k] = base[k];
        const dim3 grid(8 * UB * ((2 * p.ncl + 7) / 8));
        const size_t lds = gru_gates_lds_bytes(H, Tmax);
        OCRS_HIP(hipMemsetAsync(d_sync, 0, gru_persistent_sync_words(M) * sizeof(uint32_t), s));
        if (H == 256) launch_gates<256>(fast, grid, lds, s, p);
        else if (H == 128) launch_gates<128>(fast, grid, lds, s, p);
        else launch_gates<64>(fast, grid, lds, s, p);
        return true;
    }
    if (!gru_plan(M, Tmax, H, &p.ncl, gru_resident_capacity(H, false, gru_general_lds_bytes(H, Tmax)))) return false;
    gru_assign_tiles(h_Tm, M, p.ncl, p.tiles);
    for (int i = 0; i < 16 * p.ncl; i++) p.tbase[i] = p.tiles[i] >= 0 ? base[p.tiles[i]] : 0;
    const dim3 grid(8 * UB * ((2 * p.ncl + 7) / 8));
    if (grid.x > (unsigned)kMaxGrid) return false;
    const size_t lds = gru_general_lds_bytes(H, Tmax);
    OCRS_HIP(hipMemsetAsync(d_sync, 0, gru_persistent_sync_words(M) * sizeof(uint32_t), s));
    if (H == 256) launch_general<256>(fast, grid, lds, s, p);
    else if (H == 128) launch_general<128>(fast, grid, lds, s, p);
    else launch_general<64>(fast, grid, lds, s, p);
    return true;
}

}
}
```

ocrs_amd/csrc/kernels_nn.hip:

```cpp
#include "common.hpp"
#include "kernels.hpp"
#include "split_mfma.hpp"
#include "spec_math.hpp"

namespace ocrs {
namespace k {

typedef float f32x16 __attribute__((ext_vector_type(16)));

constexpr int GEMM_BK = 32;

template <int NT, bool IM2COL, bool CONVT>
__global__ void __launch_bounds__(256) gemm_mfma_kernel(GemmDesc d) {
    extern __shared__ __attribute__((aligned(16))) float lds_b[];
    constexpr int BN = 32 * NT;
    const int tid = threadIdx.x;
    const int lane = tid & 63;
    const int wave = tid >> 6;
    const int half = lane >> 5;
    const int l31 = lane & 31;
    const int z = blockIdx.z;
    const float* __restrict__ A = d.A + (int64_t)z * d.strideA;
    const float* __restrict__ B = d.B + (int64_t)z * d.strideB;
    const float* __restrict__ bias = d.bias ? d.bias + (int64_t)z * d.strideBias : nullptr;
// ... 876 lines not shown
        const int64_t pix = i / ct;
        float v;
        if (ch < cs) {
            v = skip[pix * cs + ch];
        } else {
            const int ox = (int)(pix % sw);
            const int oy = (int)((pix / sw) % sh);
            const int64_t img = pix / ((int64_t)sw * sh);
            const int iy = oy - py, ix = ox - px;
            v = ((unsigned)iy < (unsigned)h && (unsigned)ix < (unsigned)w) ? x[((img * h + iy) * w + ix) * cx + (ch - cs)] : 0.0f;
        }
        y[i] = v;
    }
}

void padcat(const float* skip, int n, int sh, int sw, int cs, const float* x, int h, int w, int cx, float* y,
            hipStream_t s) {
    int64_t total = (int64_t)n * sh * sw * (cs + cx);
    int grid = (int)((total + 255) / 256 < 16384 ? (total + 255) / 256 : 16384);
    if (grid < 1) grid = 1;
    hipLaunchKernelGGL(padcat_kernel, dim3(grid), dim3(256), 0, s, skip, n, sh, sw, cs, x, h, w, cx, y);
}

__global__ void __launch_bounds__(256) sigmoid_kernel(const float* __restrict__ x, float* __restrict__ y, int64_t count) {
    for (int64_t i = (int64_t)blockIdx.x * blockDim.x + threadIdx.x; i < count; i += (int64_t)gridDim.x * blockDim.x)
        y[i] = spec_sigmoidf(x[i]);
}

void sigmoid(const float* x, float* y, int64_t count, hipStream_t s) {
    int grid = (int)((count + 255) / 256 < 16384 ? (count + 255) / 256 : 16384);
    if (grid < 1) grid = 1;
    hipLaunchKernelGGL(sigmoid_kernel, dim3(grid), dim3(256), 0, s, x, y, count);
}

__global__ void __launch_bounds__(256)
conv1x1_cout1_kernel(const float* __restrict__ x, int64_t pixels, int cin, const float* __restrict__ wt,
                     const float* __restrict__ bias, int relu, int do_sigmoid, float* __restrict__ y) {
    for (int64_t p = (int64_t)blockIdx.x * blockDim.x + threadIdx.x; p < pixels; p += (int64_t)gridDim.x * blockDim.x) {
        float acc = bias[0];
        const float* xp = x + p * cin;
        if ((cin & 3) == 0) {
            for (int c = 0; c < cin; c += 4) {
                float4 v = *reinterpret_cast<const float4*>(xp + c);
                acc = fmaf(v.x, wt[c], acc);
                acc = fmaf(v.y, wt[c + 1], acc);
                acc = fmaf(v.z, wt[c + 2], acc);
                acc = fmaf(v.w, wt[c + 3], acc);
            }
        } else {
            for (int c = 0; c < cin; c++) acc = fmaf(xp[c], wt[c], acc);
        }
        if (relu) acc = acc > 0.0f ? acc : 0.0f;
        y[p] = do_sigmoid ? spec_sigmoidf(acc) : acc;
    }
}

void conv1x1_cout1(const float* x, int64_t pixels, int cin, const float* wt, const float* bias, int relu, int do_sigmoid,
                   float* y, hipStream_t s) {
    int grid = (int)((pixels + 255) / 256 < 16384 ? (pixels + 255) / 256 : 16384);
    if (grid < 1) grid = 1;
    hipLaunchKernelGGL(conv1x1_cout1_kernel, dim3(grid), dim3(256), 0, s, x, pixels, cin, wt, bias, relu, do_sigmoid, y);
}

__global__ void __launch_bounds__(256) to_seq_kernel(const float* __restrict__ x, int n, int w, int c, float* __restrict__ y) {
    const int64_t total = (int64_t)n * w * c;
    for (int64_t i = (int64_t)blockIdx.x * blockDim.x + threadIdx.x; i < total; i += (int64_t)gridDim.x * blockDim.x) {
        const int ch = (int)(i % c);
        const int64_t r = i / c;
        const int b = (int)(r % n);
        const int t = (int)(r / n);
        y[i] = x[((int64_t)b * w + t) * c + ch];
    }
}

void to_seq(const float* x, int n, int w, int c, float* y, hipStream_t s) {
    int64_t total = (int64_t)n * w * c;
    int grid = (int)((total + 255) / 256 < 16384 ? (total + 255) / 256 : 16384);
    if (grid < 1) grid = 1;
    hipLaunchKernelGGL(to_seq_kernel, dim3(grid), dim3(256), 0, s, x, n, w, c, y);
}

__global__ void __launch_bounds__(256)
gru_gates_kernel(const float* __restrict__ gx, const float* __restrict__ gh, float* __restrict__ h,
                 float* __restrict__ y, int T, int N, int H, int step) {
    const int dir = blockIdx.y;
    const int t = dir ? T - 1 - step : step;
    const int64_t total = (int64_t)N * H;
    const float* gxp = gx + (int64_t)dir * T * N * 3 * H + (int64_t)t * N * 3 * H;
    const float* ghp = gh + (int64_t)dir * N * 3 * H;
    float* hp = h + (int64_t)dir * N * H;
    for (int64_t i = (int64_t)blockIdx.x * blockDim.x + threadIdx.x; i < total; i += (int64_t)gridDim.x * blockDim.x) {
        const int j = (int)(i % H);
        const int64_t b = i / H;
        const float* gxr = gxp + b * 3 * H;
        const float* ghr = ghp + b * 3 * H;
        float r = spec_sigmoidf(gxr[j] + ghr[j]);
        float z = spec_sigmoidf(gxr[H + j] + ghr[H + j]);
        float nn = spec_tanhf(fmaf(r, ghr[2 * H + j], gxr[2 * H + j]));
        float hprev = hp[i];
        float hn = fmaf(z, hprev - nn, nn);
        hp[i] = hn;
        y[((int64_t)t * N + b) * 2 * H + (int64_t)dir * H + j] = hn;
    }
}

void gru_gates(const float* gx, const float* gh, float* h, float* y, int T, int N, int H, int step, hipStream_t s) {
    int64_t total = (int64_t)N * H;
    int grid = (int)((total + 255) / 256 < 4096 ? (total + 255) / 256 : 4096);
    if (grid < 1) grid = 1;
    hipLaunchKernelGGL(gru_gates_kernel, dim3(grid, 2), dim3(256), 0, s, gx, gh, h, y, T, N, H, step);
}

constexpr int LSM_ROWS = 64;

__device__ __forceinline__ void log_softmax_argmax_body(const float* __restrict__ logits, int64_t rows, int c,
                                                        const uint8_t* __restrict__ excl, float* __restrict__ logp,
                                                        int32_t* __restrict__ labels, float* __restrict__ maxlp) {
    extern __shared__ float tile[];
    const int cp = (c & 1) ? c : c + 1;
    const int64_t r0 = (int64_t)blockIdx.x * LSM_ROWS;
    const int nrows = (int)min((int64_t)LSM_ROWS, rows - r0);
    for (int i = threadIdx.x; i < nrows * c; i += LSM_ROWS) {
        int rr = i / c, cc = i - rr * c;
        tile[rr * cp + cc] = logits[r0 * c + i];
    }
    __syncthreads();
    if ((int)threadIdx.x < nrows) {
        float* row = tile + threadIdx.x * cp;
        float m = row[0];
        for (int j = 1; j < c; j++) m = row[j] > m ? row[j] : m;
        float ssum = 0.0f;
        for (int j = 0; j < c; j++) ssum = ssum + spec_expf(row[j] - m);
        const float lse = m + spec_logf(ssum);
        const float ninf = -__builtin_huge_valf();
        int best = 0;
        float bv = row[0] - lse;
        row[0] = bv;
        if (excl && excl[0]) bv = ninf;
        for (int j = 1; j < c; j++) {
            float v = row[j] - lse;
            row[j] = v;
            if (excl && excl[j]) v = ninf;
            if (v > bv) { bv = v; best = j; }
        }
        if (labels) labels[r0 + threadIdx.x] = best;
        if (maxlp) maxlp[r0 + threadIdx.x] = bv;
    }
    __syncthreads();
    if (logp)
        for (int i = threadIdx.x; i < nrows * c; i += LSM_ROWS) {
            int rr = i / c, cc = i - rr * c;
            logp[r0 * c + i] = tile[rr * cp + cc];
        }
}

__global__ void __launch_bounds__(LSM_ROWS)
log_softmax_argmax_kernel(const float* __restrict__ logits, int64_t rows, int c, const uint8_t* __restrict__ excl,
                          float* __restrict__ logp, int32_t* __restrict__ labels) {
    log_softmax_argmax_body(logits, rows, c, excl, logp, labels, nullptr);
}

__global__ void __launch_bounds__(LSM_ROWS)
log_softmax_argmax_max_kernel(const float* __restrict__ logits, int64_t rows, int c, const uint8_t* __restrict__ excl,
                              float* __restrict__ logp, int32_t* __restrict__ labels, float* __restrict__ maxlp) {
    log_softmax_argmax_body(logits, rows, c, excl, logp, labels, maxlp);
}

bool log_softmax_argmax(const float* logits, int64_t rows, int c, const uint8_t* d_excluded, float* logp,
                        int32_t* labels, hipStream_t s, float* maxlp) {
    if (rows <= 0) return true;
    int cp = (c & 1) ? c : c + 1;
    size_t lds = (size_t)LSM_ROWS * cp * sizeof(float);
    if (lds > 160 * 1024) return false;
    if (lds > 64 * 1024) {
        static std::atomic<uint64_t> lds_ok{0}, lds_ok_max{0};
        if (maxlp) allow_dynamic_lds(reinterpret_cast<const void*>(&log_softmax_argmax_max_kernel), lds_ok_max);
        else allow_dynamic_lds(reinterpret_cast<const void*>(&log_softmax_argmax_kernel), lds_ok);
    }
    int grid = (int)((rows + LSM_ROWS - 1) / LSM_ROWS);
    if (maxlp)
        hipLaunchKernelGGL(log_softmax_argmax_max_kernel, dim3(grid), dim3(LSM_ROWS), lds, s, logits, rows, c, d_excluded,
                           logp, labels, maxlp);
    else
        hipLaunchKernelGGL(log_softmax_argmax_kernel, dim3(grid), dim3(LSM_ROWS), lds, s, logits, rows, c, d_excluded, logp,
                           labels);
    return true;
}

__global__ void __launch_bounds__(256)
to_seq_packed_kernel(const float* __restrict__ x, int n, int T, int c, const int32_t* __restrict__ pos,
                     const int32_t* __restrict__ off, float* __restrict__ y) {
    const int64_t total = (int64_t)n * T * c;
    for (int64_t i = (int64_t)blockIdx.x * blockDim.x + threadIdx.x; i < total; i += (int64_t)gridDim.x * blockDim.x) {
        const int ch = (int)(i % c);
        const int64_t r = i / c;
        const int t = (int)(r % T);
        const int line = (int)(r / T);
        y[((int64_t)off[t] + pos[line]) * c + ch] = x[i];
    }
}

void to_seq_packed(const float* x, int n, int T, int c, const int32_t* d_pos, const int32_t* d_off, float* y,
                   hipStream_t s) {
    int64_t total = (int64_t)n * T * c;
    if (total <= 0) return;
    int grid = (int)((total + 255) / 256 < 16384 ? (total + 255) / 256 : 16384);
    hipLaunchKernelGGL(to_seq_packed_kernel, dim3(grid), dim3(256), 0, s, x, n, T, c, d_pos, d_off, y);
}

__global__ void __launch_bounds__(256)
gru_gates_packed_kernel(const float* __restrict__ gx, const float* __restrict__ gh, float* __restrict__ h,
                        float* __restrict__ y, const int32_t* __restrict__ Tm, const int32_t* __restrict__ off,
                        int64_t R, int Mcap, int active, int H, int step) {
    const int dir = blockIdx.y;
    const int64_t total = (int64_t)active * H;
    const float* gxd = gx + (int64_t)dir * R * 3 * H;
    const float* ghd = gh + (int64_t)dir * Mcap * 3 * H;
    float* hd = h + (int64_t)dir * Mcap * H;
    for (int64_t i = (int64_t)blockIdx.x * blockDim.x + threadIdx.x; i < total; i += (int64_t)gridDim.x * blockDim.x) {
        const int j = (int)(i % H);
        const int m = (int)(i / H);
        const int t = dir ? Tm[m] - 1 - step : step;
        const int64_t row = (int64_t)off[t] + m;
        const float* gxr = gxd + row * 3 * H;
        const float* ghr = ghd + (int64_t)m * 3 * H;
        float r = spec_sigmoidf(gxr[j] + ghr[j]);
        float z = spec_sigmoidf(gxr[H + j] + ghr[H + j]);
        float nn = spec_tanhf(fmaf(r, ghr[2 * H + j], gxr[2 * H + j]));
        float hprev = hd[i];
        float hn = fmaf(z, hprev - nn, nn);
        hd[i] = hn;
        y[row * 2 * H + (int64_t)dir * H + j] = hn;
    }
}

typedef float f32x4 __attribute__((ext_vector_type(4)));

template <int H>
__global__ void __launch_bounds__(256)
gru_step_fused_kernel(const float* __restrict__ gx, const float* __restrict__ wh, const float* __restrict__ bh,
                      const float* __restrict__ hT_in, float* __restrict__ hT_out, float* __restrict__ y,
                      const int32_t* __restrict__ Tm, const int32_t* __restrict__ off, int64_t R, int Mcap, int active,
                      int step) {
    extern __shared__ __attribute__((aligned(16))) float lds_w[];
    const int dir = blockIdx.z;
    const int j0 = blockIdx.y * 16;
    const int tid = threadIdx.x;
    const int lane = tid & 63, wave = tid >> 6;
    const int row0 = blockIdx.x * 64 + wave * 16;
    const float* __restrict__ whd = wh + (int64_t)dir * H * 3 * H;
    const float* __restrict__ bhd = bh + (int64_t)dir * 3 * H;
    const float* __restrict__ hin = hT_in + (int64_t)dir * H * Mcap;
    float* __restrict__ hout = hT_out + (int64_t)dir * H * Mcap;
    const float* __restrict__ gxd = gx + (int64_t)dir * R * 3 * H;

    const int i16 = lane & 15, kq = lane >> 4;
    const bool wave_active = row0 < active;

    float areg[H / 4];
    const int arow = min(row0 + i16, Mcap - 1);
    if (wave_active) {
        const float* ap = hin + (int64_t)kq * Mcap + arow;
#pragma unroll
        for (int s4 = 0; s4 < H / 4; s4++) areg[s4] = ap[(int64_t)s4 * 4 * Mcap];
    }
    const int j = j0 + i16;
    const int mbase = row0 + kq * 4;
    float gxr_[4], gxz_[4], gxn_[4], hprev_[4];
    int64_t yrow[4];
    bool rok[4];
#pragma unroll
    for (int r = 0; r < 4; r++) {
        const int m = mbase + r;
        rok[r] = wave_active && m < active;
        gxr_[r] = gxz_[r] = gxn_[r] = hprev_[r] = 0.0f;
        yrow[r] = 0;
        if (rok[r]) {
            const int t = dir ? Tm[m] - 1 - step : step;
            const int64_t row = (int64_t)off[t] + m;
            const float* g = gxd + row * 3 * H;
            gxr_[r] = g[j];
            gxz_[r] = g[H + j];
            gxn_[r] = g[2 * H + j];
            hprev_[r] = hin[(int64_t)j * Mcap + m];
            yrow[r] = row;
        }
    }
    for (int i = tid; i < H * 12; i += 256) {
        const int k = i / 12, q = i - k * 12;
        const int g = q >> 2, c4 = (q & 3) * 4;
        const float4 v = *reinterpret_cast<const float4*>(whd + (int64_t)k * 3 * H + g * H + j0 + c4);
        *reinterpret_cast<float4*>(&lds_w[k * 48 + g * 16 + c4]) = v;
    }
    __syncthreads();
    if (!wave_active) return;

    f32x4 acc_r, acc_z, acc_n;
    {
        const float br = bhd[j0 + i16], bz = bhd[H + j0 + i16], bn = bhd[2 * H + j0 + i16];
        for (int r = 0; r < 4; r++) { acc_r[r] = br; acc_z[r] = bz; acc_n[r] = bn; }
    }
    const float* bp = &lds_w[kq * 48 + i16];
#pragma unroll
    for (int s4 = 0; s4 < H / 4; s4++) {
        const float a = areg[s4];
        const float* b = bp + s4 * 4 * 48;
        acc_r = __builtin_amdgcn_mfma_f32_16x16x4f32(a, b[0], acc_r, 0, 0, 0);
        acc_z = __builtin_amdgcn_mfma_f32_16x16x4f32(a, b[16], acc_z, 0, 0, 0);
        acc_n = __builtin_amdgcn_mfma_f32_16x16x4f32(a, b[32], acc_n, 0, 0, 0);
    }
    float hnew[4];
#pragma unroll
    for (int r = 0; r < 4; r++) {
        float hn = 0.0f;
        if (rok[r]) {
            const float rg = spec_sigmoidf(gxr_[r] + acc_r[r]);
            const float zg = spec_sigmoidf(gxz_[r] + acc_z[r]);
            const float ng = spec_tanhf(fmaf(rg, acc_n[r], gxn_[r]));
            hn = fmaf(zg, hprev_[r] - ng, ng);
            y[yrow[r] * 2 * H + (int64_t)dir * H + j] = hn;
        }
        hnew[r] = hn;
    }
    float* hp = hout + (int64_t)j * Mcap + mbase;
    if (mbase + 3 < Mcap) {
        *reinterpret_cast<float4*>(hp) = make_float4(hnew[0], hnew[1], hnew[2], hnew[3]);
    } else {
        for (int r = 0; r < 4 && mbase + r < Mcap; r++) hp[r] = hnew[r];
    }
}

bool gru_step_fused(const float* gx, const float* wh, const float* bh, const float* hT_in, float* hT_out, float* y,
                    const int32_t* d_Tm, const int32_t* d_off, int64_t R, int Mcap, int active, int H, int step,
                    hipStream_t s) {
    if (active <= 0) return true;
    dim3 grid((active + 63) / 64, H / 16, 2);
    size_t lds = (size_t)H * 48 * sizeof(float);
    if (H == 256)
        hipLaunchKernelGGL((gru_step_fused_kernel<256>), grid, dim3(256), lds, s, gx, wh, bh, hT_in, hT_out, y, d_Tm, d_off,
                           R, Mcap, active, step);
    else if (H == 128)
        hipLaunchKernelGGL((gru_step_fused_kernel<128>), grid, dim3(256), lds, s, gx, wh, bh, hT_in, hT_out, y, d_Tm, d_off,
                           R, Mcap, active, step);
    else if (H == 64)
        hipLaunchKernelGGL((gru_step_fused_kernel<64>), grid, dim3(256), lds, s, gx, wh, bh, hT_in, hT_out, y, d_Tm, d_off, R,
                           Mcap, active, step);
    else
        return false;
    return true;
}

void gru_gates_packed(const float* gx, const float* gh, float* h, float* y, const int32_t* d_Tm, const int32_t* d_off,
                      int64_t R, int Mcap, int active, int H, int step, hipStream_t s) {
    int64_t total = (int64_t)active * H;
    if (total <= 0) return;
    int grid = (int)((total + 255) / 256 < 4096 ? (total + 255) / 256 : 4096);
    hipLaunchKernelGGL(gru_gates_packed_kernel, dim3(grid, 2), dim3(256), 0, s, gx, gh, h, y, d_Tm, d_off, R, Mcap, active,
                       H, step);
}

__global__ void __launch_bounds__(64)
ctc_collapse_packed_kernel(const int32_t* __restrict__ labels, const int32_t* __restrict__ Tm,
                           const int32_t* __restrict__ off, int M, int Tmax, uint32_t* __restrict__ out_labels,
                           uint32_t* __restrict__ out_pos, int32_t* __restrict__ out_count) {
    const int m = blockIdx.x * blockDim.x + threadIdx.x;
    if (m >= M) return;
    const int T = Tm[m];
    int last = 0, cnt = 0;
    for (int t = 0; t < T; t++) {
        int l = labels[(int64_t)off[t] + m];
        if (l == last) continue;
        last = l;
        if (l > 0) {
            out_labels[(int64_t)m * Tmax + cnt] = (uint32_t)l;
            out_pos[(int64_t)m * Tmax + cnt] = (uint32_t)t;
            cnt++;
        }
    }
    out_count[m] = cnt;
}

void ctc_collapse_packed(const int32_t* labels, const int32_t* d_Tm, const int32_t* d_off, int M, int Tmax,
                         uint32_t* out_labels, uint32_t* out_pos, int32_t* out_count, hipStream_t s) {
    if (M <= 0) return;
    hipLaunchKernelGGL(ctc_collapse_packed_kernel, dim3((M + 63) / 64), dim3(64), 0, s, labels, d_Tm, d_off, M, Tmax,
                       out_labels, out_pos, out_count);
}

constexpr int CTC_U = 16;

__global__ void __launch_bounds__(64)
ctc_collapse_scored_packed_kernel(const int32_t* __restrict__ labels, const float* __restrict__ maxlp,
                                  const int32_t* __restrict__ Tm, const int32_t* __restrict__ off, int M, int Tmax,
                                  uint32_t* __restrict__ out_labels, uint32_t* __restrict__ out_pos,
                                  float* __restrict__ out_logp, int32_t* __restrict__ out_count,
                                  double* __restrict__ out_score) {
    const int m = blockIdx.x * blockDim.x + threadIdx.x;
    const int T = m < M ? Tm[m] : 0;
    int Tw = T;
#pragma unroll
    for (int d = 32; d >= 1; d >>= 1) Tw = max(Tw, __shfl_xor(Tw, d));
    int last = 0, cnt = 0;
    double s = 0.0;
    const int64_t base = (int64_t)m * Tmax;
    for (int t0 = 0; t0 < Tw; t0 += CTC_U) {
        int l[CTC_U];
        float v[CTC_U];
#pragma unroll
        for (int u = 0; u < CTC_U; u++) {
            const int t = t0 + u;
            l[u] = 0;
            v[u] = 0.0f;
            if (t < T) {
                const int64_t r = (int64_t)off[t] + m;
                l[u] = labels[r];
                v[u] = maxlp[r];
            }
        }
#pragma unroll
        for (int u = 0; u < CTC_U; u++) {
            const int t = t0 + u;
            if (t >= T) break;
            s += (double)v[u];
            if (l[u] == last) continue;
            last = l[u];
            if (l[u] > 0) {
                out_labels[base + cnt] = (uint32_t)l[u];
                out_pos[base + cnt] = (uint32_t)t;
                out_logp[base + cnt] = v[u];
                cnt++;
            }
        }
    }
    if (m < M) {
        out_count[m] = cnt;
        out_score[m] = s;
    }
}

void ctc_collapse_scored_packed(const int32_t* labels, const float* maxlp, const int32_t* d_Tm, const int32_t* d_off, int M,
                                int Tmax, uint32_t* out_labels, uint32_t* out_pos, float* out_logp, int32_t* out_count,
// ... 57 lines not shown
```

ocrs_amd/csrc/model.cpp:

```cpp
#include "model.hpp"

#include <cstdio>
#include <functional>
#include <map>
#include <mutex>

#include "kernels.hpp"

namespace ocrs {

namespace {
#pragma pack(push, 1)
struct FileHeader {
    char magic[8];
    uint32_t version, kind;
    int64_t input_shape[4];
    uint32_t n_ops, n_slots, out_slot, reserved;
    uint64_t blob_floats;
};
struct FileOp {
    uint32_t type;
    int32_t in0, in1, out, relu, kh, kw, cin, cout, hidden;
    uint32_t n_w, reserved;
    struct { uint64_t off, cnt; } w[8];
// ... 31 lines not shown
    if (memcmp(hd.magic, "OCRSMDL1", 8) != 0 || hd.version != 1) fail(OCRS_ERR_IO, "not an OCRSMDL1 model file");
    if (hd.n_ops > (1u << 20) || hd.n_slots == 0 || hd.n_slots > (1u << 20) || hd.out_slot >= hd.n_slots)
        fail(OCRS_ERR_IO, "model file header out of range (%u ops, %u slots, output slot %u)", hd.n_ops, hd.n_slots, hd.out_slot);
    const size_t table = sizeof(FileHeader) + (size_t)hd.n_ops * sizeof(FileOp);
    if (len < table || hd.blob_floats > (len - table) / sizeof(float)) fail(OCRS_ERR_IO, "model file truncated");
    const float* blob = reinterpret_cast<const float*>(static_cast<const char*>(data) + table);

    auto m = std::make_unique<HipModel>();
    m->kind = hd.kind;
    for (int i = 0; i < 4; i++) m->input_shape[i] = hd.input_shape[i];
    m->n_slots = hd.n_slots;
    m->out_slot = hd.out_slot;

    std::vector<float> slab(blob, blob + hd.blob_floats);
    auto pad16 = [&]() { while (slab.size() % 4) slab.push_back(0.f); };
    pad16();
    struct Fix { size_t op; int which; size_t off; };
    std::vector<Fix> fixes;
    std::vector<FileOp> fops(hd.n_ops);
    for (uint32_t i = 0; i < hd.n_ops; i++) {
        memcpy(&fops[i], static_cast<const char*>(data) + sizeof(FileHeader) + (size_t)i * sizeof(FileOp), sizeof(FileOp));
        const FileOp& f = fops[i];
        if (f.type >= OP_COUNT || f.n_w > 8) fail(OCRS_ERR_IO, "bad op record %u", i);
        for (uint32_t j = 0; j < f.n_w; j++)
            if (f.w[j].off > hd.blob_floats || f.w[j].cnt > hd.blob_floats - f.w[j].off)
                fail(OCRS_ERR_IO, "weight reference out of range in op %u", i);
        {
            const int64_t ns = hd.n_slots;
            const bool two_in = f.type == OP_PADCAT;
            if (f.in0 < 0 || f.in0 >= ns || f.out <= 0 || f.out >= ns || (two_in ? (f.in1 < 0 || f.in1 >= ns) : false) ||
                (!two_in && f.in1 >= ns))
                fail(OCRS_ERR_IO, "slot index out of range in op %u", i);
            auto want = [&](uint32_t j, int64_t cnt) {
                if (j >= f.n_w || cnt < 0 || (int64_t)f.w[j].cnt != cnt)
                    fail(OCRS_ERR_IO, "op %u (%s): weight tensor %u has %llu floats, the op's shape needs %lld", i,
                         kOpNames[f.type], j, j < f.n_w ? (unsigned long long)f.w[j].cnt : 0ull, (long long)cnt);
            };
            auto pos = [&](int64_t v, const char* what) {
                if (v <= 0 || v > (1 << 20)) fail(OCRS_ERR_IO, "op %u (%s): bad %s %lld", i, kOpNames[f.type], what, (long long)v);
            };
            switch (f.type) {
                case OP_CONV: pos(f.kh, "kh"); pos(f.kw, "kw"); pos(f.cin, "cin"); pos(f.cout, "cout");
                    want(0, (int64_t)f.kh * f.kw * f.cin * f.cout); want(1, f.cout); break;
                case OP_DWCONV3: pos(f.cin, "channels"); want(0, 9LL * f.cin); want(1, f.cin); break;
                case OP_MAXPOOL: case OP_AVGPOOL: pos(f.kh, "kh"); pos(f.kw, "kw"); break;
                case OP_CONVT2: pos(f.cin, "cin"); pos(f.cout, "cout"); want(0, 4LL * f.cin * f.cout); want(1, f.cout); break;
                case OP_GRU: pos(f.cin, "input size"); pos(f.hidden, "hidden size");
                    if (f.n_w != 8) fail(OCRS_ERR_IO, "GRU op %u needs 8 weight tensors", i);
                    for (uint32_t d = 0; d < 2; d++) {
                        want(4 * d + 0, 3LL * f.cin * f.hidden); want(4 * d + 1, 3LL * f.hidden);
                        want(4 * d + 2, 3LL * f.hidden * f.hidden); want(4 * d + 3, 3LL * f.hidden);
                    }
                    break;
                case OP_LINEAR: pos(f.cin, "cin"); pos(f.cout, "cout"); want(0, (int64_t)f.cin * f.cout); want(1, f.cout); break;
                default: break;
            }
        }
        GraphOp op{};
        op.type = f.type; op.in0 = f.in0; op.in1 = f.in1; op.out = f.out;
        op.relu = f.relu; op.kh = f.kh; op.kw = f.kw; op.cin = f.cin; op.cout = f.cout; op.hidden = f.hidden;
        for (uint32_t j = 0; j < f.n_w; j++) op.wcount[j] = f.w[j].cnt;
        if (f.type == OP_CONVT2) {
            const float* w = blob + f.w[0].off;
            const float* b = blob + f.w[1].off;
            fixes.push_back({i, 0, slab.size()});
            for (int ci = 0; ci < f.cin; ci++)
                for (int q = 0; q < 4; q++)
                    for (int co = 0; co < f.cout; co++) slab.push_back(w[((size_t)q * f.cin + ci) * f.cout + co]);
            pad16();
            fixes.push_back({i, 1, slab.size()});
            for (int q = 0; q < 4; q++)
                for (int co = 0; co < f.cout; co++) slab.push_back(b[co]);
            pad16();
        } else if (f.type == OP_GRU) {
            if (f.n_w != 8) fail(OCRS_ERR_IO, "GRU op %u needs 8 weight tensors", i);
            for (int part = 0; part < 4; part++) {
                fixes.push_back({i, part, slab.size()});
                for (int d = 0; d < 2; d++) {
                    const float* src = blob + f.w[4 * d + part].off;
                    slab.insert(slab.end(), src, src + f.w[4 * d + part].cnt);
                }
                pad16();
            }
        }
        m->ops.push_back(op);
    }
    {
        std::vector<int64_t> chans(hd.n_slots, -1);
        chans[0] = 1;
        for (uint32_t i = 0; i < hd.n_ops; i++) {
            const FileOp& f = fops[i];
            auto in = [&](int32_t sl) {
                if (chans[sl] < 0)
                    fail(OCRS_ERR_IO, "op %u (%s): input slot %d is not written by an earlier op", i, kOpNames[f.type], sl);
                return chans[sl];
            };
            const int64_t c0 = in(f.in0);
            auto need = [&](int64_t want, const char* what) {
                if (c0 != want)
                    fail(OCRS_ERR_IO, "op %u (%s): %s is %lld but input slot %d carries %lld channels", i, kOpNames[f.type], what,
                         (long long)want, f.in0, (long long)c0);
            };
            int64_t co = c0;
            switch (f.type) {
                case OP_CONV: case OP_CONVT2: case OP_LINEAR: need(f.cin, "cin"); co = f.cout; break;
                case OP_DWCONV3: need(f.cin, "channels"); break;
                case OP_GRU: need(f.cin, "input size"); co = 2LL * f.hidden; break;
                case OP_PADCAT: co = c0 + in(f.in1); break;
                default: break;
            }
            if (co > (1 << 24)) fail(OCRS_ERR_IO, "op %u (%s): %lld output channels", i, kOpNames[f.type], (long long)co);
            chans[f.out] = co;
        }
        if (chans[hd.out_slot] < 0) fail(OCRS_ERR_IO, "the output slot %u is not written by any op", hd.out_slot);
    }
    DeviceScope bind(device);
    m->device = ctx().device;
    m->weights = DevBuf(slab.size() * sizeof(float));
    OCRS_HIP(hipMemcpy(m->weights.p, slab.data(), slab.size() * sizeof(float), hipMemcpyHostToDevice));
    const float* base = m->weights.as<float>();
    for (uint32_t i = 0; i < hd.n_ops; i++)
        for (uint32_t j = 0; j < fops[i].n_w; j++) m->ops[i].w[j] = base + fops[i].w[j].off;
    for (const Fix& fx : fixes) {
        GraphOp& op = m->ops[fx.op];
        const float* p = base + fx.off;
        if (fx.which == 0) op.aux0 = p;
        else if (fx.which == 1) op.aux1 = p;
        else if (fx.which == 2) op.aux2 = p;
        else op.aux3 = p;
    }
    for (uint32_t i = 0; i < hd.n_ops; i++) {
        GraphOp& op = m->ops[i];
        if (m->kind == 1 && op.type == OP_CONV && op.kh == 3 && op.kw == 3 && (op.cin % 32) == 0 && (op.cout % 128) == 0) {
            std::vector<uint16_t> img;
            k::split_weights(slab.data() + fops[i].w[0].off, 9 * op.cin, op.cout, op.cout, &img);
            m->tapes.emplace_back(img.size() * sizeof(uint16_t));
            OCRS_HIP(hipMemcpy(m->tapes.back().p, img.data(), img.size() * sizeof(uint16_t), hipMemcpyHostToDevice));
            op.wsplit = m->tapes.back().as<uint16_t>();
        }
        if (m->kind == 1 && op.type == OP_CONV && op.kh == 3 && op.kw == 3 && op.cin == 32 && op.cout == 64) {
            std::vector<uint16_t> img;
            k::conv12_split_weights(slab.data() + fops[i].w[0].off, &img);
            m->tapes.emplace_back(img.size() * sizeof(uint16_t));
            OCRS_HIP(hipMemcpy(m->tapes.back().p, img.data(), img.size() * sizeof(uint16_t), hipMemcpyHostToDevice));
            op.wsplit = m->tapes.back().as<uint16_t>();
        }
    }
    for (const Fix& fx : fixes) {
        GraphOp& op = m->ops[fx.op];
        if (fx.which != 0 || op.type != OP_GRU || (op.cin % 64) != 0 || ((3 * op.hidden) % 128) != 0) continue;
        std::vector<uint16_t> both;
        for (int dir = 0; dir < 2; dir++) {
            std::vector<uint16_t> img;
            k::split_weights(slab.data() + fx.off + (size_t)dir * op.cin * 3 * op.hidden, op.cin, 3 * op.hidden, 3 * op.hidden, &img);
            both.insert(both.end(), img.begin(), img.end());
        }
        m->tapes.emplace_back(both.size() * sizeof(uint16_t));
        OCRS_HIP(hipMemcpy(m->tapes.back().p, both.data(), both.size() * sizeof(uint16_t), hipMemcpyHostToDevice));
        op.wsplit = m->tapes.back().as<uint16_t>();
    }
    for (size_t i = 0; i + 1 < m->ops.size(); i++) {
        GraphOp& a = m->ops[i];
        GraphOp& b = m->ops[i + 1];
        if (a.type == OP_CONV && a.cout == 1 && a.kh == 1 && a.kw == 1 && b.type == OP_SIGMOID && b.in0 == a.out) {
            bool other_use = false;
            for (size_t j = i + 2; j < m->ops.size(); j++)
                if (m->ops[j].in0 == a.out || m->ops[j].in1 == a.out) other_use = true;
            if (!other_use && (uint32_t)a.out != m->out_slot) b.fused_into_prev = true;
        }
    }
    for (size_t i = 0; i + 1 < m->ops.size(); i++) {
        GraphOp& a = m->ops[i];
        GraphOp& b = m->ops[i + 1];
        if (a.type == OP_DWCONV3 && b.type == OP_CONV && b.kh == 1 && b.kw == 1 && b.in0 == a.out && b.cin == a.cin &&
            k::dwpw_fused_supported(a.cin, b.cout) && (uint32_t)a.out != m->out_slot) {
            bool other_use = false;
            for (size_t j = i + 2; j < m->ops.size(); j++)
                if (m->ops[j].in0 == a.out || m->ops[j].in1 == a.out) other_use = true;
            if (!other_use) { a.fuse_next_pw = true; b.done_by_prev = true; }
        }
    }
    for (size_t i = 0; i + 1 < m->ops.size(); i++) {
        GraphOp& a = m->ops[i];
        GraphOp& b = m->ops[i + 1];
        if (a.type == OP_PADCAT && b.type == OP_DWCONV3 && b.in0 == a.out && (uint32_t)a.out != m->out_slot) {
            bool other_use = false;
            for (size_t j = i + 2; j < m->ops.size(); j++)
                if (m->ops[j].in0 == a.out || m->ops[j].in1 == a.out) other_use = true;
            if (!other_use) { a.cat_into_next = true; b.reads_cat = true; }
        }
    }
    {
        auto& ops = m->ops;
        const int n = (int)ops.size();
        auto uses = [&](int slot) {
            int u = 0;
            for (const GraphOp& o : ops) u += (o.in0 == slot) + (o.in1 == slot);
            return u + ((uint32_t)slot == m->out_slot ? 1 : 0);
        };
        auto pw11 = [](const GraphOp& o) { return o.type == OP_CONV && o.kh == 1 && o.kw == 1; };
        for (int i = 0; i + 3 < n; i++) {
            DcBlock b;
            int j = i;
            if (ops[j].type == OP_CONVT2 && j + 1 < n && ops[j + 1].type == OP_PADCAT && ops[j + 1].in1 == ops[j].out &&
                uses(ops[j].out) == 1 && uses(ops[j + 1].out) == 1) {
                b.convt = j; b.cat = j + 1;
                j += 2;
            }
            if (j + 3 >= n) continue;
            const GraphOp &d1 = ops[j], &p1 = ops[j + 1], &d2 = ops[j + 2], &p2 = ops[j + 3];
            if (d1.type != OP_DWCONV3 || !pw11(p1) || d2.type != OP_DWCONV3 || !pw11(p2)) continue;
            if (b.cat >= 0 && d1.in0 != ops[b.cat].out) continue;
// ... 290 lines not shown
                          [&] { k::conv1x1_cout1(x, px, op.cin, op.w[0], op.w[1], op.relu, next_sigmoid ? 1 : 0, y, st); });
                } else if (op.kh == 1 && op.kw == 1 && (op.cin % 4) == 0) {
                    k::GemmDesc d{};
                    d.A = x; d.lda = op.cin; d.B = op.w[0]; d.ldb = op.cout; d.bias = op.w[1];
                    d.C = y; d.ldc = op.cout; d.M = (int)px; d.N = op.cout; d.K = op.cin; d.relu = op.relu;
                    timed(KC_GEMM_POINTWISE, cflops, cbytes, [&] { k::gemm(d, st); });
                } else if (op.kh == 3 && op.kw == 3 && (op.cin % 32) == 0) {
                    k::GemmDesc d{};
                    d.A = x; d.B = op.w[0]; d.ldb = op.cout; d.bias = op.w[1];
                    d.C = y; d.ldc = op.cout; d.M = (int)px; d.N = op.cout; d.K = 9 * op.cin; d.relu = op.relu;
                    d.im2col = 1; d.H = a.h; d.W = a.w; d.Cin = op.cin;
                    timed(KC_GEMM_CONV3X3, cflops, cbytes, [&] { k::gemm(d, st); });
                } else if ((op.cout % 4) == 0) {
                    timed(KC_CONV_DIRECT, cflops, cbytes, [&] {
                        k::conv_direct(x, a.n, a.h, a.w, op.cin, op.w[0], op.w[1], op.kh, op.kw, op.cout, op.relu, y, st);
                    });
                } else {
                    fail(OCRS_ERR_RUN_FAILED, "model run failed: unsupported conv shape %dx%d %d->%d", op.kh, op.kw,
                         op.cin, op.cout);
                }
                break;
            }
            case OP_DWCONV3:
                if (op.reads_cat && i > 0 && cat_fused(i - 1)) {
                    const GraphOp& cat = ops[i - 1];
                    const TensorShape sk = shp[cat.in0], up = shp[cat.in1];
                    if ((sk.c % 4) == 0 && (up.c % 4) == 0) {
                        timed(KC_DWCONV3X3, 18.0 * a.count(), 8.0 * a.count(), [&] {
                            k::dwconv3x3_cat(ptr[cat.in0], sk.n, sk.h, sk.w, sk.c, ptr[cat.in1], up.h, up.w, up.c, op.w[0],
                                             op.w[1], op.relu, y, st);
                        });
                    } else {
                        auto tmp = get((size_t)a.count());
                        timed(KC_PADCAT, 0, 8.0 * a.count(), [&] {
                            k::padcat(ptr[cat.in0], sk.n, sk.h, sk.w, sk.c, ptr[cat.in1], up.h, up.w, up.c, tmp.first, st);
                        });
                        timed(KC_DWCONV3X3, 18.0 * a.count(), 8.0 * a.count(),
                              [&] { k::dwconv3x3(tmp.first, a.n, a.h, a.w, a.c, op.w[0], op.w[1], op.relu, y, st); });
                        free_local.emplace(tmp.second, tmp.first);
                    }
                    for (int sl : {cat.in0, cat.in1})
                        if (sl > 0 && last_use[sl] == (int)i && ptr[sl] && cap[sl]) {
                            free_local.emplace(cap[sl], ptr[sl]);
                            ptr[sl] = nullptr;
                            cap[sl] = 0;
                        }
                    break;
                }
                timed(KC_DWCONV3X3, 18.0 * a.count(), 8.0 * a.count(),
                      [&] { k::dwconv3x3(x, a.n, a.h, a.w, a.c, op.w[0], op.w[1], op.relu, y, st); });
                break;
            case OP_MAXPOOL:
                timed(KC_POOL, 0, 4.0 * (a.count() + o.count()), [&] { k::maxpool(x, a.n, a.h, a.w, a.c, op.kh, op.kw, y, st); });
                break;
            case OP_AVGPOOL:
                timed(KC_POOL, 0, 4.0 * (a.count() + o.count()), [&] { k::avgpool(x, a.n, a.h, a.w, a.c, op.kh, op.kw, y, st); });
                break;
            case OP_CONVT2: {
                k::GemmDesc d{};
                d.A = x; d.lda = op.cin; d.B = op.aux0; d.ldb = 4 * op.cout; d.bias = op.aux1;
                d.C = y; d.M = (int)((int64_t)a.n * a.h * a.w); d.N = 4 * op.cout; d.K = op.cin;
                d.convt = 1; d.H = a.h; d.W = a.w; d.Cout = op.cout;
                timed(KC_GEMM_CONVT, 2.0 * d.M * op.cin * op.cout * 4, 4.0 * (a.count() + o.count()) + wbytes(op, 0),
                      [&] { k::gemm(d, st); });
                break;
            }
            case OP_PADCAT: {
                const TensorShape b = shp[op.in1];
                timed(KC_PADCAT, 0, 8.0 * o.count(),
                      [&] { k::padcat(x, a.n, a.h, a.w, a.c, ptr[op.in1], b.h, b.w, b.c, y, st); });
                break;
            }
            case OP_SIGMOID: timed(KC_OTHER, 0, 8.0 * a.count(), [&] { k::sigmoid(x, y, a.count(), st); }); break;
            case OP_TOSEQ:
                if (a.h != 1) fail(OCRS_ERR_RUN_FAILED, "model run failed: TOSEQ expects height 1, got %d", a.h);
                timed(KC_OTHER, 0, 8.0 * a.count(), [&] { k::to_seq(x, a.n, a.w, a.c, y, st); });
                break;
            case OP_GRU: {
                const int T = a.n, N = a.h, I = a.c, H = op.hidden;
                auto gx = get((size_t)2 * T * N * 3 * H);
                auto gh = get((size_t)2 * N * 3 * H);
                auto hs = get((size_t)2 * N * H);
                OCRS_HIP(hipMemsetAsync(hs.first, 0, (size_t)2 * N * H * sizeof(float), st));
                k::GemmDesc d{};
                d.A = x; d.lda = I; d.B = op.aux0; d.ldb = 3 * H; d.bias = op.aux1; d.C = gx.first; d.ldc = 3 * H;
                d.M = T * N; d.N = 3 * H; d.K = I; d.batch = 2;
                d.strideA = 0; d.strideB = (int64_t)I * 3 * H; d.strideBias = 3 * H; d.strideC = (int64_t)T * N * 3 * H;
                timed(KC_GEMM_GRU_INPUT, 2.0 * 2 * d.M * (double)d.N * d.K,
                      4.0 * ((double)a.count() + 2.0 * d.M * d.N + 2.0 * d.K * d.N), [&] { k::gemm(d, st); });
                k::GemmDesc r{};
                r.A = hs.first; r.lda = H; r.B = op.aux2; r.ldb = 3 * H; r.bias = op.aux3; r.C = gh.first; r.ldc = 3 * H;
                r.M = N; r.N = 3 * H; r.K = H; r.batch = 2;
                r.strideA = (int64_t)N * H; r.strideB = (int64_t)H * 3 * H; r.strideBias = 3 * H; r.strideC = (int64_t)N * 3 * H;
                for (int step = 0; step < T; step++) {
                    timed(KC_GEMM_GRU_HIDDEN, 2.0 * 2 * r.M * (double)r.N * r.K,
                          4.0 * 2 * ((double)r.M * r.K + (double)r.M * r.N + (double)r.K * r.N), [&] { k::gemm(r, st); });
                    timed(KC_GRU_GATES, 0, 4.0 * 2 * N * (double)H * 9,
                          [&] { k::gru_gates(gx.first, gh.first, hs.first, y, T, N, H, step, st); });
                }
                free_local.emplace(gx.second, gx.first);
                free_local.emplace(gh.second, gh.first);
                free_local.emplace(hs.second, hs.first);
                break;
            }
            case OP_LINEAR: {
                k::GemmDesc d{};
                d.A = x; d.lda = op.cin; d.B = op.w[0]; d.ldb = op.cout; d.bias = op.w[1];
                d.C = y; d.ldc = op.cout; d.M = (int)((int64_t)a.n * a.h * a.w); d.N = op.cout; d.K = op.cin;
                d.relu = op.relu;
                timed(KC_GEMM_LINEAR, 2.0 * d.M * (double)d.N * d.K, 4.0 * ((double)a.count() + o.count()) + wbytes(op, 0),
                      [&] { k::gemm(d, st); });
                break;
            }
            case OP_LOGSOFTMAX:
                timed(KC_LOGSOFTMAX_ARGMAX, 0, 4.0 * a.count() * (y ? 2.0 : 1.0), [&] {
                    if (!k::log_softmax_argmax(x, (int64_t)a.n * a.h * a.w, a.c, is_final_logsoftmax ? d_excluded : nullptr, y,
                                               is_final_logsoftmax ? d_labels : nullptr, st))
                        fail(OCRS_ERR_CAPACITY, "LogSoftmax over %d classes exceeds the kernel's LDS staging (max ~630)", a.c);
                });
                break;
            default: fail(OCRS_ERR_RUN_FAILED, "model run failed: bad op");
        }
        }
        if (print_timing) OCRS_HIP(hipEventRecord(ev[i + 1], st));
        for (int sl : {op.in0, op.in1}) {
            if (sl > 0 && last_use[sl] == (int)i && ptr[sl] && cap[sl]) {
                free_local.emplace(cap[sl], ptr[sl]);
                ptr[sl] = nullptr;
                cap[sl] = 0;
            }
        }
    }
    if (timers && cur_stage >= 0) timers->end(stage_token, st);
    OCRS_HIP(hipGetLastError());

    if (print_timing) {
        OCRS_HIP(hipStreamSynchronize(st));
        float total = 0.f;
        for (size_t i = 0; i < n_run; i++) {
            float ms = 0.f;
            (void)hipEventElapsedTime(&ms, ev[i], ev[i + 1]);
            total += ms;
            const TensorShape o = shp[ops[i].out];
            printf("%-10s [%d,%d,%d,%d] %.3fms\n", kOpNames[ops[i].type], o.n, o.h, o.w, o.c, ms);
        }
        printf("total %.3fms\n", total);
        for (auto& e : ev) (void)hipEventDestroy(e);
    }
    return ptr[ret_slot];
}

float* HipModel::run_prefix_ragged(Workspace& ws, hipStream_t exec, const std::vector<PackedGroup>& groups,
                                   const PackedPlan& plan, int h, int ts, StageTimers* timers, int* feat_c,
                                   const std::function<void()>& before_launch, const OpRange* range) const {
    const int G = (int)groups.size();
    if (G == 0 || ts <= 0) return nullptr;
    for (int i = 0; i < ts; i++) {
        const GraphOp& op = ops[i];
        if (op.in0 != (i == 0 ? 0 : ops[i - 1].out)) return nullptr;
        if (op.type == OP_CONV) {
            if (op.kh != 3 || op.kw != 3 || !op.relu) return nullptr;
            if (op.cin == 1) {
                if (i + 1 >= ts || ops[i + 1].type != OP_MAXPOOL || ops[i + 1].kh != 2 || ops[i + 1].kw != 2) return nullptr;
                if (op.cout > 64 || op.cout < 4 || (op.cout & (op.cout - 1)) != 0) return nullptr;
            } else if ((op.cin % 32) != 0 || op.cout < 64 || (op.cout % 4) != 0) {
                return nullptr;
            }
        } else if (op.type != OP_MAXPOOL && op.type != OP_AVGPOOL) {
            return nullptr;
        }
    }
    {
        int hh = h;
        for (int i = 0; i < ts; i++) {
            if (ops[i].type == OP_CONV && ops[i].cin != 1 && (hh % 4) != 0) return nullptr;
            if (ops[i].type == OP_MAXPOOL || ops[i].type == OP_AVGPOOL) hh /= ops[i].kh;
        }
    }
    for (int g = 0; g + 1 < G && !(range && range->first > 0); g++)
        if (groups[g].d_batch + (size_t)groups[g].n * h * groups[g].w != groups[g + 1].d_batch) return nullptr;

// ... 320 lines not shown
                                     float** d_logp, float* d_maxlp, OpRange* range) const {
    const int ts = packed_split();
    if (ts < 0) fail(OCRS_ERR_RUN_FAILED, "model run failed: graph is not <conv stack> TOSEQ GRU* LINEAR LOGSOFTMAX");
    const int first = range ? range->first : 0, last = range ? range->last : (int)ops.size() - 1;
    hipStream_t st = ws.s();
    auto timed = [&](int cls, double flops, double bytes, auto&& launch) {
        int tok = timers ? timers->kbegin(cls, st, flops, bytes) : -1;
        launch();
        if (tok >= 0) timers->end(tok, st);
    };
    const int64_t R = plan.R;
    const int M = plan.M;

    float* X = nullptr;
    int C0 = 0;
    if (first <= ts) {
        std::unique_lock<std::mutex> heavy(ctx().heavy_phase, std::defer_lock);
        const hipStream_t conv = ws.stream.conv_stream();
        try {
            X = run_prefix_ragged(ws, conv, groups, plan, h, ts, timers, &C0, [&] { heavy.lock(); }, range);
        } catch (...) {
            hipEvent_t e = nullptr;
            if (hipEventCreateWithFlags(&e, hipEventDisableTiming) == hipSuccess) {
                ws.events.push_back(e);
                if (hipEventRecord(e, conv) != hipSuccess || hipStreamWaitEvent(ws.s(), e, 0) != hipSuccess)
                    (void)hipStreamSynchronize(conv);
            } else {
                (void)hipStreamSynchronize(conv);
            }
            throw;
        }
    }
    if (range && first <= ts) {
        if (!X) fail(OCRS_ERR_INVALID_ARGUMENT, "op range: this model's conv stack has no ragged form");
        if (last < ts) {
            range->out = X;
            range->out_c = C0;
            return 0;
        }
    }
    if (!X && first <= ts)
    for (const PackedGroup& g : groups) {
        TensorShape fs;
        float* feat = run_device(ws, g.d_batch, g.n, h, g.w, &fs, timers, nullptr, nullptr, true, false, ts);
        if (fs.h != 1) fail(OCRS_ERR_RUN_FAILED, "model run failed: TOSEQ expects height 1, got %d", fs.h);
        if (!X) {
            C0 = fs.c;
            X = ws.alloc_n<float>((size_t)R * C0);
        }
        int tok = timers ? timers->begin(ST_REC_CONV, st, 0) : -1;
        timed(KC_OTHER, 0, 8.0 * fs.count(), [&] { k::to_seq_packed(feat, g.n, fs.w, fs.c, g.d_pos, plan.d_off, X, st); });
        if (tok >= 0) timers->end(tok, st);
    }
    if (!X && first <= ts) return 0;

    const float* cur = first <= ts ? X : range->seq_in;
    int curC = first <= ts ? C0 : range->in_c;
    int classes = 0;
    int gru_layer = 0;
    float* gx_buf = nullptr;
    size_t gx_cap = 0;
    void* hx_buf = nullptr;
    size_t hx_cap = 0;
    for (int i = std::max(ts + 1, first); i <= last; i++) {
        const GraphOp& op = ops[i];
        if (op.type == OP_GRU) {
            const int H = op.hidden, I = op.cin;
            if (I != curC) fail(OCRS_ERR_RUN_FAILED, "model run failed: GRU input size %d != %d", I, curC);
            int tok = timers ? timers->begin(ST_REC_GRU, st, 0) : -1;
            const size_t gx_floats = (size_t)2 * R * 3 * H;
            if (gx_floats > gx_cap) { gx_buf = ws.alloc_n<float>(gx_floats); gx_cap = gx_floats; }
            float* gx = gx_buf;
            float* y = ws.alloc_n<float>((size_t)R * 2 * H);
            const bool fused = (H == 256 || H == 128 || H == 64);
            const bool persistent = fused && gru_mode() == GRU_PERSISTENT && k::gru_persistent_supported(plan.h_Tm.data(), M, plan.Tmax, R, H);
            const int np = option(OPT_NUMERICS) == 1 ? 3 : option(OPT_NUMERICS) == 2 ? 2 : 0;
            const bool split = persistent && np != 0 && k::gru_split_supported(plan.h_Tm.data(), M, plan.Tmax, R, H, np);
            const size_t hx_bytes = split ? k::gru_split_exchange_bytes(plan.h_Tm.data(), M, H, np) : persistent ? k::gru_persistent_exchange_bytes(plan.h_Tm.data(), M, H) : 0;
            if (hx_bytes > hx_cap) { hx_buf = ws.alloc(hx_bytes); hx_cap = hx_bytes; }
            uint16_t* hx = split ? static_cast<uint16_t*>(hx_buf) : nullptr;
            float* hxf = persistent && !split ? static_cast<float*>(hx_buf) : nullptr;
            if (split) OCRS_HIP(k::gru_split_prepare(hx, plan.h_Tm.data(), M, H, np, st));
            else if (persistent) OCRS_HIP(k::gru_persistent_prepare(hxf, plan.h_Tm.data(), M, H, st));
            k::GemmDesc d{};
            d.A = cur; d.lda = I; d.B = op.aux0; d.ldb = 3 * H; d.bias = op.aux1; d.C = gx; d.ldc = 3 * H;
            d.M = (int)R; d.N = 3 * H; d.K = I; d.batch = 2;
            d.strideA = 0; d.strideB = (int64_t)I * 3 * H; d.strideBias = 3 * H; d.strideC = R * 3 * H;
            d.Bsplit = op.wsplit; d.strideBsplit = (int64_t)(3 * H / 128) * (I / 16) * 3 * 128 * 16;
            const double gx_flops = 2.0 * 2 * R * (double)d.N * d.K, gx_bytes = 4.0 * ((double)R * I + 2.0 * R * d.N + 2.0 * d.K * d.N);
            timed(KC_GEMM_GRU_INPUT, gx_flops, gx_bytes, [&] { k::gemm(d, st); });
            if (range && range->gx_only && i == last) {
                range->out = gx;
                range->out_c = 3 * H;
                return 0;
            }
            bool ran_persistent = false;
            if (persistent) {
                uint32_t* d_sync = ws.alloc_n<uint32_t>(k::gru_persistent_sync_words(M));
                double fl = 0.0;
                for (int step = 0; step < plan.Tmax; step++) fl += 2.0 * 2 * plan.active[step] * 3.0 * H * H;
                {
                    DeviceContext& dc = ctx();
                    std::lock_guard<std::mutex> g(dc.rec_phase);
                    hipStream_t rs = ws.stream.recurrent_stream();
                    hipEvent_t ready = ws.make_event(), done = ws.make_event();
                    OCRS_HIP(hipEventRecord(ready, st));
                    OCRS_HIP(hipStreamWaitEvent(rs, ready, 0));
                    int ktok = timers ? timers->kbegin(KC_GEMM_GRU_HIDDEN, rs, fl, 4.0 * ((double)R * (2.0 * 3 * H + 2.0 * 2 * H) + 2.0 * 3 * H * H)) : -1;
                    ran_persistent = split ? k::gru_persistent_split(gx, op.aux2, op.aux3, y, hx, plan.d_Tm, plan.d_off, plan.h_Tm.data(), R, M, plan.Tmax, H, np, d_sync, rs)
                                           : k::gru_persistent(gx, op.aux2, op.aux3, y, hxf, plan.d_Tm, plan.d_off, plan.h_Tm.data(), R, M, plan.Tmax, H, d_sync, rs);
                    if (ktok >= 0) timers->end(ktok, rs);
                    if (ran_persistent && plan.h_status && gru_layer < 8)
                        ws.download(plan.h_status + gru_layer, d_sync + k::gru_persistent_sync_words(M) - 1, sizeof(uint32_t), rs);
                    OCRS_HIP(hipEventRecord(done, rs));
                    OCRS_HIP(hipStreamWaitEvent(st, done, 0));
                }
            }
            if (ran_persistent) {
            } else if (fused) {
                const int Mcap = (M + 3) & ~3;
                float* hT0 = ws.alloc_n<float>((size_t)2 * H * Mcap);
                float* hT1 = ws.alloc_n<float>((size_t)2 * H * Mcap);
                OCRS_HIP(hipMemsetAsync(hT0, 0, (size_t)2 * H * Mcap * sizeof(float), st));
                for (int step = 0; step < plan.Tmax; step++) {
                    const int act = plan.active[step];
                    if (act <= 0) break;
                    const float* hin = (step & 1) ? hT1 : hT0;
                    float* hout = (step & 1) ? hT0 : hT1;
                    timed(KC_GEMM_GRU_HIDDEN, 2.0 * 2 * act * 3.0 * H * H,
                          4.0 * 2 * ((double)act * H * 2 + (double)act * 3 * H + 3.0 * H * H + (double)act * H), [&] {
                              if (!k::gru_step_fused(gx, op.aux2, op.aux3, hin, hout, y, plan.d_Tm, plan.d_off, R, Mcap, act, H, step, st))
                                  fail(OCRS_ERR_RUN_FAILED, "model run failed: no fused GRU step kernel for hidden size %d", H);
                          });
                }
            } else {
                float* gh = ws.alloc_n<float>((size_t)2 * M * 3 * H);
                float* hs = ws.alloc_n<float>((size_t)2 * M * H);
                OCRS_HIP(hipMemsetAsync(hs, 0, (size_t)2 * M * H * sizeof(float), st));
                k::GemmDesc r{};
                r.A = hs; r.lda = H; r.B = op.aux2; r.ldb = 3 * H; r.bias = op.aux3; r.C = gh; r.ldc = 3 * H;
                r.N = 3 * H; r.K = H; r.batch = 2;
                r.strideA = (int64_t)M * H; r.strideB = (int64_t)H * 3 * H; r.strideBias = 3 * H; r.strideC = (int64_t)M * 3 * H;
                for (int step = 0; step < plan.Tmax; step++) {
                    const int act = plan.active[step];
                    if (act <= 0) break;
                    r.M = act;
                    timed(KC_GEMM_GRU_HIDDEN, 2.0 * 2 * act * (double)r.N * r.K,
                          4.0 * 2 * ((double)act * r.K + (double)act * r.N + (double)r.K * r.N), [&] { k::gemm(r, st); });
                    timed(KC_GRU_GATES, 0, 4.0 * 2 * act * (double)H * 9, [&] {
                        k::gru_gates_packed(gx, gh, hs, y, plan.d_Tm, plan.d_off, R, M, act, H, step, st);
                    });
                }
            }
            if (tok >= 0) timers->end(tok, st);
            gru_layer++;
            cur = y;
            curC = 2 * H;
        } else if (op.type == OP_LINEAR) {
            if (op.cin != curC) fail(OCRS_ERR_RUN_FAILED, "model run failed: Linear input size %d != %d", op.cin, curC);
            int tok = timers ? timers->begin(ST_REC_HEAD, st, 0) : -1;
            float* y = ws.alloc_n<float>((size_t)R * op.cout);
            k::GemmDesc d{};
            d.A = cur; d.lda = op.cin; d.B = op.w[0]; d.ldb = op.cout; d.bias = op.w[1];
            d.C = y; d.ldc = op.cout; d.M = (int)R; d.N = op.cout; d.K = op.cin; d.relu = op.relu;
            timed(KC_GEMM_LINEAR, 2.0 * R * (double)d.N * d.K, 4.0 * ((double)R * (op.cin + op.cout)) + 4.0 * op.wcount[0],
                  [&] { k::gemm(d, st); });
            if (tok >= 0) timers->end(tok, st);
            cur = y;
            curC = op.cout;
        } else {
            int tok = timers ? timers->begin(ST_REC_HEAD, st, 0) : -1;
            float* lp = nullptr;
            if (d_logp || range) {
                lp = ws.alloc_n<float>((size_t)R * curC);
                if (d_logp) *d_logp = lp;
            }
            timed(KC_LOGSOFTMAX_ARGMAX, 0, 4.0 * R * curC * (lp ? 2.0 : 1.0),
                  [&] {
                      if (!k::log_softmax_argmax(cur, R, curC, d_excluded, lp, d_labels, st, d_maxlp))
                          fail(OCRS_ERR_CAPACITY, "LogSoftmax over %d classes exceeds the kernel's LDS staging (max ~630)", curC);
                  });
            if (tok >= 0) timers->end(tok, st);
            classes = curC;
            if (range) cur = lp;
        }
    }
    if (range) {
        range->out = cur;
        range->out_c = curC;
    }
    OCRS_HIP(hipGetLastError());
    return classes;
}

}
```

ocrs_amd/csrc/model.hpp:

```cpp
#pragma once
#include <functional>
#include <memory>
#include <string>
#include <vector>

#include "common.hpp"

namespace ocrs {

enum OpType : uint32_t {
    OP_CONV = 0, OP_DWCONV3, OP_MAXPOOL, OP_AVGPOOL, OP_CONVT2, OP_PADCAT, OP_SIGMOID, OP_TOSEQ, OP_GRU, OP_LINEAR,
    OP_LOGSOFTMAX, OP_COUNT
};

struct GraphOp {
    uint32_t type;
    int32_t in0, in1, out;
    int32_t relu, kh, kw, cin, cout, hidden;
    const float* w[8] = {nullptr};
    size_t wcount[8] = {0};
    const float* aux0 = nullptr;
    const float* aux1 = nullptr;
    const float* aux2 = nullptr;
    const float* aux3 = nullptr;
    const uint16_t* wsplit = nullptr;
    bool fused_into_prev = false;
    bool fuse_next_pw = false;
    bool done_by_prev = false;
    bool cat_into_next = false;
    bool reads_cat = false;
    int dc_block = -1;
};

struct DcBlock {
    int first = -1, last = -1;
    int convt = -1, cat = -1, dw1 = -1, pw1 = -1, dw2 = -1, pw2 = -1, pool = -1, fin = -1, sig = -1;
    int cs = 0, cx = 0, cmid = 0, cout = 0;
    const float* tape = nullptr;
    int tape_len = 0;
    const float* rtape = nullptr;
    int rtape_len = 0;
};

struct TensorShape {
    int n = 0, h = 0, w = 0, c = 0;
    bool seq = false;
    int64_t count() const { return (int64_t)n * h * w * c; }
};

struct ModelBase {
    virtual ~ModelBase() = default;
    int device = -1;
    int64_t input_shape[4] = {-1, -1, -1, -1};
    virtual bool is_callback() const = 0;
};

struct CallbackModel : ModelBase {
    ocrs_model_run_fn fn = nullptr;
    void* user = nullptr;
    bool is_callback() const override { return true; }
    void run(const float* input, const int64_t in_shape[4], std::vector<float>& out, int64_t out_shape[4],
             int* out_ndim) const;
};

struct HipModel : ModelBase {
    uint32_t kind = 0;
    std::vector<GraphOp> ops;
    std::vector<DcBlock> dc_blocks;
    uint32_t n_slots = 0, out_slot = 0;
    DevBuf weights;
    std::vector<DevBuf> tapes;
    bool is_callback() const override { return false; }

    static std::unique_ptr<HipModel> load(const void* data, size_t len, int device = -1);

    TensorShape infer(int n, int h, int w, std::vector<TensorShape>* slots = nullptr) const;
    double flops(int n, int h, int w) const;

    float* run_device(Workspace& ws, const float* d_in, int n, int h, int w, TensorShape* out_shape,
                      StageTimers* timers, const uint8_t* d_excluded = nullptr, int32_t* d_labels = nullptr,
                      bool want_logp = true, bool print_timing = false, int stop_before = -1,
                      hipStream_t exec = nullptr ) const;

    int packed_split() const;
    struct PackedGroup {
        const float* d_batch;
        int n, w;
        const int32_t* d_pos;
    };
    struct PackedPlan {
        int M = 0, Tmax = 0;
        int64_t R = 0;
        const int32_t* d_Tm = nullptr;
        const int32_t* d_off = nullptr;
        std::vector<int> active;
        std::vector<int32_t> h_Tm;
        std::vector<int32_t> h_off;
        uint32_t* h_status = nullptr;
    };
    struct OpRange {
        int first = 0, last = 0;
        bool gx_only = false;
        const float* seq_in = nullptr;
        int in_c = 0;
        const float* out = nullptr;
        int out_c = 0;
    };
// ... 15 lines not shown
```

Baseline: 273.7.

## Interleave GRU input-gate columns per 16-unit block and refetch only missing state pieces

Adds a blocked column layout for the GRU input-projection output (gx), where each 16-unit block stores its r, z and n gates contiguously. At load time the input weights and biases are permuted into this layout so the GEMM writes it directly, and every GRU gate and step kernel indexes gx through the new layout. This should make each tile's gate loads more local. The persistent kernel also stops loading a separate copy of its own previous-state piece: it picks that piece out of the already-loaded h array, and while spin-waiting it reloads only the pieces still unwritten. The cost is a second copy of the input weights on the device, plus a new option and ABI helper.

Measured after the change: 272.4. No clear change (-0.5%).

```diff
diff --git a/include/ocrs_amd.h b/include/ocrs_amd.h
--- a/include/ocrs_amd.h
+++ b/include/ocrs_amd.h
@@ -45,6 +45,8 @@
 
 OCRS_API ocrs_status ocrs_gru_tile_plan(const int32_t* lengths_desc, size_t n_lines, int hidden, int32_t* n_clusters, int32_t* waves,
                                         int16_t* tiles);
+
+OCRS_API ocrs_status ocrs_gru_gx_column(int hidden, int blocked, int gate, int unit, int32_t* column, int32_t* natural_of_column);
 
 OCRS_API ocrs_status ocrs_coalescer_selftest(int n_threads, int requests_per_thread, int max_active, int max_pages,
                                              long window_us, int fail_every, uint64_t out[5]);
diff --git a/ocrs_amd/_lib.py b/ocrs_amd/_lib.py
--- a/ocrs_amd/_lib.py
+++ b/ocrs_amd/_lib.py
@@ -58,7 +58,7 @@
     "ocrs_engine_prepare_recognition_input", "ocrs_text_item_rotated_rect", "ocrs_rotated_rect_corners", "ocrs_engine_get_text", "ocrs_device_malloc", "ocrs_device_free",
     "ocrs_device_upload", "ocrs_device_synchronize", "ocrs_device_measure_peaks", "ocrs_engine_enable_timing", "ocrs_stage_count",
     "ocrs_stage_name", "ocrs_engine_stage_times", "ocrs_kernel_class_count", "ocrs_kernel_class_name",
-    "ocrs_engine_kernel_stats", "ocrs_engine_set_kernel_timing_mask", "ocrs_gru_tile_plan", "ocrs_host_malloc", "ocrs_host_free", "ocrs_engine_prepare_input_batch",
+    "ocrs_engine_kernel_stats", "ocrs_engine_set_kernel_timing_mask", "ocrs_gru_tile_plan", "ocrs_gru_gx_column", "ocrs_host_malloc", "ocrs_host_free", "ocrs_engine_prepare_input_batch",
     "ocrs_get_device", "ocrs_model_load_file_on_device", "ocrs_model_load_bytes_on_device", "ocrs_model_device", "ocrs_engine_device",
     "ocrs_engine_group_new", "ocrs_engine_group_free", "ocrs_engine_group_size", "ocrs_engine_group_member", "ocrs_group_deal",
     "ocrs_group_prepare_input_batch", "ocrs_group_prepare_input_device_batch", "ocrs_group_detect_words_batch",
diff --git a/ocrs_amd/csrc/abi.cpp b/ocrs_amd/csrc/abi.cpp
--- a/ocrs_amd/csrc/abi.cpp
+++ b/ocrs_amd/csrc/abi.cpp
@@ -54,6 +54,16 @@
         if (!k::gru_tile_plan(lengths_desc, (int)n_lines, hidden, &ncl, waves, tiles))
             fail(OCRS_ERR_CAPACITY, "no persistent-kernel plan for this shape (the engine then runs the recurrence as one fused launch per time step)");
         *n_clusters = ncl;
+    });
+}
+
+ocrs_status ocrs_gru_gx_column(int hidden, int blocked, int gate, int unit, int32_t* column, int32_t* natural_of_column) {
+    return guarded([&] {
+        if (!column || !natural_of_column || hidden < 1 || hidden > (1 << 20) || gate < 0 || gate > 2 || unit < 0 || unit >= hidden ||
+            (blocked != 0 && !gru_gx_blockable(hidden)))
+            fail(OCRS_ERR_INVALID_ARGUMENT, "bad argument");
+        *column = gru_gx_col(hidden, blocked != 0, gate, unit);
+        *natural_of_column = blocked ? gru_gx_to_natural(hidden, *column) : *column;
     });
 }
 
diff --git a/ocrs_amd/csrc/common.cpp b/ocrs_amd/csrc/common.cpp
--- a/ocrs_amd/csrc/common.cpp
+++ b/ocrs_amd/csrc/common.cpp
@@ -408,6 +408,7 @@
     {"gru_mode", "OCRS_GRU_MODE", GRU_PERSISTENT},
     {"gru_gates", "OCRS_GRU_GATES", 1},
     {"gru_local", "OCRS_GRU_LOCAL", 1},
+    {"gru_gx_blocked", "OCRS_GRU_GX_BLOCKED", 1},
     {"det_fuse", "OCRS_DET_FUSE", 1},
     {"det_stream", "OCRS_DET_STREAM", 1},
     {"det_rows", "OCRS_DET_ROWS", 1},
@@ -425,7 +426,7 @@
 };
 struct OptRange { long lo, hi; long also[4]; };
 const OptRange kOptRanges[OPT_COUNT] = {
-    {0, 1, {}}, {0, 1, {}}, {0, 1, {}}, {0, 2, {}}, {0, 1, {8, 14, 32}}, {0, 1, {8, 14, 20, 32}}, {0, 1, {}}, {0, 1, {}}, {0, 1, {}}, {0, 1, {}},
+    {0, 1, {}}, {0, 1, {}}, {0, 1, {}}, {0, 1, {}}, {0, 2, {}}, {0, 1, {8, 14, 32}}, {0, 1, {8, 14, 20, 32}}, {0, 1, {}}, {0, 1, {}}, {0, 1, {}}, {0, 1, {}},
     {1, 1024, {}},
     {0, 2, {}}, {0, 64, {}}, {1, 4096, {}}, {0, 10000000, {}}, {0, 4096, {}}, {0, INT64_MAX, {}},
 };
diff --git a/ocrs_amd/csrc/common.hpp b/ocrs_amd/csrc/common.hpp
--- a/ocrs_amd/csrc/common.hpp
+++ b/ocrs_amd/csrc/common.hpp
@@ -139,7 +139,7 @@
 inline HostPool& host_pool() { return ctx().host_pool; }
 inline hipStream_t heavy_stream() { return ctx().heavy_stream(); }
 
-enum Option { OPT_GRU_MODE = 0, OPT_GRU_GATES, OPT_GRU_LOCAL, OPT_DET_FUSE, OPT_DET_STREAM, OPT_DET_ROWS, OPT_CCL_QUAD,
+enum Option { OPT_GRU_MODE = 0, OPT_GRU_GATES, OPT_GRU_LOCAL, OPT_GRU_GX_BLOCKED, OPT_DET_FUSE, OPT_DET_STREAM, OPT_DET_ROWS, OPT_CCL_QUAD,
               OPT_CONV12_FUSE, OPT_CONV_FLAT, OPT_BEAM_GPU, OPT_DET_TILE_BATCH, OPT_PUBLIC_COUNT,
               OPT_NUMERICS = OPT_PUBLIC_COUNT,
               OPT_COALESCE, OPT_COALESCE_PAGES, OPT_COALESCE_WINDOW_US,
diff --git a/ocrs_amd/csrc/gru_layout.hpp b/ocrs_amd/csrc/gru_layout.hpp
--- /dev/null
+++ b/ocrs_amd/csrc/gru_layout.hpp
@@ -0,0 +1,23 @@
+#pragma once
+
+#if defined(__HIPCC__)
+#define OCRS_GRU_LAYOUT_FN __host__ __device__ inline
+#else
+#define OCRS_GRU_LAYOUT_FN inline
+#endif
+
+namespace ocrs {
+
+OCRS_GRU_LAYOUT_FN bool gru_gx_blockable(int H) { return H > 0 && (H % 16) == 0; }
+
+OCRS_GRU_LAYOUT_FN int gru_gx_col(int H, bool blocked, int gate, int unit) {
+    return blocked ? (unit >> 4) * 48 + gate * 16 + (unit & 15) : gate * H + unit;
+}
+
+OCRS_GRU_LAYOUT_FN int gru_gx_to_blocked(int H, int natural_col) { return gru_gx_col(H, true, natural_col / H, natural_col % H); }
+OCRS_GRU_LAYOUT_FN int gru_gx_to_natural(int H, int blocked_col) {
+    const int ub = blocked_col / 48, r = blocked_col % 48;
+    return gru_gx_col(H, false, r >> 4, ub * 16 + (r & 15));
+}
+
+}
diff --git a/ocrs_amd/csrc/kernels.hpp b/ocrs_amd/csrc/kernels.hpp
--- a/ocrs_amd/csrc/kernels.hpp
+++ b/ocrs_amd/csrc/kernels.hpp
@@ -3,6 +3,8 @@
 #include <hip/hip_runtime.h>
 
 #include <cstdint>
+
+#include "gru_layout.hpp"
 
 namespace ocrs {
 namespace jpeg { struct Coefficients; }
@@ -112,23 +114,23 @@
 void conv1x1_cout1(const float* x, int64_t pixels, int cin, const float* wt, const float* bias, int relu, int do_sigmoid,
                    float* y, hipStream_t s);
 void to_seq(const float* x, int n, int w, int c, float* y, hipStream_t s);
-void gru_gates(const float* gx, const float* gh, float* h, float* y, int T, int N, int H, int step, hipStream_t s);
+void gru_gates(const float* gx, const float* gh, float* h, float* y, int T, int N, int H, int step, bool gx_blocked, hipStream_t s);
 bool log_softmax_argmax(const float* logits, int64_t rows, int c, const uint8_t* d_excluded ,
                         float* logp, int32_t* labels, hipStream_t s, float* maxlp = nullptr);
 void to_seq_packed(const float* x, int n, int T, int c, const int32_t* d_pos, const int32_t* d_off, float* y,
                    hipStream_t s);
 void gru_gates_packed(const float* gx, const float* gh, float* h, float* y, const int32_t* d_Tm, const int32_t* d_off,
-                      int64_t R, int Mcap, int active, int H, int step, hipStream_t s);
+                      int64_t R, int Mcap, int active, int H, int step, bool gx_blocked, hipStream_t s);
 bool gru_step_fused(const float* gx, const float* wh, const float* bh, const float* hT_in, float* hT_out, float* y,
                     const int32_t* d_Tm, const int32_t* d_off, int64_t R, int Mcap, int active, int H, int step,
-                    hipStream_t s);
+                    bool gx_blocked, hipStream_t s);
 size_t gru_persistent_sync_words(int M);
 size_t gru_persistent_exchange_bytes(const int32_t* h_Tm, int M, int H);
 bool gru_persistent_supported(const int32_t* h_Tm, int M, int Tmax, int64_t R, int H);
 bool gru_tile_plan(const int32_t* h_Tm, int M, int H, int* ncl, int* waves, int16_t* tiles );
 hipError_t gru_persistent_prepare(float* hx, const int32_t* h_Tm, int M, int H, hipStream_t s);
 bool gru_persistent(const float* gx, const float* wh, const float* bh, float* y, float* hx, const int32_t* d_Tm, const int32_t* d_off,
-                    const int32_t* h_Tm, int64_t R, int M, int Tmax, int H, uint32_t* d_sync, hipStream_t s);
+                    const int32_t* h_Tm, int64_t R, int M, int Tmax, int H, bool gx_blocked, uint32_t* d_sync, hipStream_t s);
 bool gru_general_tile_plan(const int32_t* h_Tm, int M, int Tmax, int H, int cap, int* ncl, int16_t* tiles , int kernel );
 size_t gru_split_exchange_bytes(const int32_t* h_Tm, int M, int H, int np);
 bool gru_split_supported(const int32_t* h_Tm, int M, int Tmax, int64_t R, int H, int np);
diff --git a/ocrs_amd/csrc/kernels_gru.hip b/ocrs_amd/csrc/kernels_gru.hip
--- a/ocrs_amd/csrc/kernels_gru.hip
+++ b/ocrs_amd/csrc/kernels_gru.hip
@@ -32,6 +32,7 @@
     int M, ncl, Tmax;
     int prio;
     int allow_local;
+    int gx_blocked;
     int16_t tiles[kMaxSlots * 4];
     int32_t tbase[kMaxSlots * 4];
     int TB;
@@ -69,7 +70,6 @@
 template <int H>
 struct Loaded {
     f32x4 h[H / 16];
-    f32x4 hp;
     f32x4 gr, gz, gn;
     uint32_t out_off;
     uint32_t hx_off;
@@ -93,26 +93,25 @@
     const uint32_t blk = (uint32_t)(dir * p.TB + tbase + s);
     L.hx_off = (blk * (H / 16) + ub) * 1024u + i16 * 64u + kq * 16u;
     if (L.active) {
-        const float* g = p.gx + ((int64_t)dir * p.R + row) * 3 * H + ub * 16 + kq * 4;
+        const float* g = p.gx + ((int64_t)dir * p.R + row) * 3 * H + gru_gx_col(H, p.gx_blocked != 0, 0, ub * 16 + kq * 4);
+        const int gs = p.gx_blocked ? 16 : H;
         L.gr = *reinterpret_cast<const f32x4*>(g);
-        L.gz = *reinterpret_cast<const f32x4*>(g + H);
-        L.gn = *reinterpret_cast<const f32x4*>(g + 2 * H);
+        L.gz = *reinterpret_cast<const f32x4*>(g + gs);
+        L.gn = *reinterpret_cast<const f32x4*>(g + 2 * gs);
         if (s > 0) L.prev_off = (blk - 1u) * (H / 16) * 1024u + i16 * 64u;
     }
 }
 
 template <int H>
-__device__ __forceinline__ void issue_state(__amdgpu_buffer_rsrc_t y, int ub, int kq, Loaded<H>& L) {
+__device__ __forceinline__ void issue_state(__amdgpu_buffer_rsrc_t y, int kq, Loaded<H>& L) {
     constexpr uint32_t kPiece = 1024u;
     if (L.has_prev) {
 #pragma unroll
         for (int j = 0; j < H / 16; j++) L.h[j] = load_bypass(y, L.prev_off + j * kPiece + kq * 16);
-        L.hp = load_bypass(y, L.prev_off + ub * kPiece + kq * 16);
     } else {
         const f32x4 zero = {0.0f, 0.0f, 0.0f, 0.0f};
 #pragma unroll
         for (int j = 0; j < H / 16; j++) L.h[j] = zero;
-        L.hp = zero;
     }
 }
 
@@ -123,14 +122,40 @@
     for (int j = 0; j < H / 16; j++)
 #pragma unroll
         for (int e = 0; e < 4; e++) mx = max(mx, __float_as_uint(L.h[j][e]));
-#pragma unroll
-    for (int e = 0; e < 4; e++) mx = max(mx, __float_as_uint(L.hp[e]));
     return !__any(mx == kUnwritten);
 }
 
 template <int H>
-__device__ __forceinline__ bool await_state(const GruParams& p, __amdgpu_buffer_rsrc_t y, int ub, int kq, Loaded<H>& L) {
+__device__ __forceinline__ uint32_t missing_pieces(const Loaded<H>& L) {
+    uint32_t miss = 0;
+#pragma unroll
+    for (int j = 0; j < H / 16; j++) {
+        const unsigned mx = max(max(__float_as_uint(L.h[j][0]), __float_as_uint(L.h[j][1])), max(__float_as_uint(L.h[j][2]), __float_as_uint(L.h[j][3])));
+        if (__any(mx == kUnwritten)) miss |= 1u << j;
+    }
+    miss = __builtin_amdgcn_readfirstlane(miss);
+    asm volatile("" : "+s"(miss));
+    return miss;
+}
+
+template <int H>
+__device__ __forceinline__ f32x4 own_piece(const Loaded<H>& L, int ub) {
+    f32x4 r = L.h[0];
+    asm volatile("" : "+s"(ub));
+#pragma unroll
+    for (int j = 1; j < H / 16; j++)
+        if (ub == j) {
+            r = L.h[j];
+            asm volatile("" : "+v"(r));
+        }
+    return r;
+}
+
+template <int H>
+__device__ __forceinline__ bool await_state(const GruParams& p, __amdgpu_buffer_rsrc_t y, int kq, Loaded<H>& L) {
+    constexpr uint32_t kPiece = 1024u;
     for (uint32_t spins = 0; !state_ready<H>(L); spins++) {
+        const uint32_t miss = missing_pieces<H>(L);
         __builtin_amdgcn_s_sleep(2);
         if (spins >= 4u) {
             const uint32_t n = spins < 36u ? (spins >> 2) : 9u;
@@ -144,7 +169,11 @@
                 return false;
             }
         }
-        issue_state<H>(y, ub, kq, L);
+#pragma unroll
+        for (int j = 0; j < H / 16; j++)
+            if (miss & (1u << j)) {
+                if (L.has_prev) L.h[j] = load_bypass(y, L.prev_off + j * kPiece + kq * 16);
+            }
     }
     return true;
 }
@@ -304,7 +333,7 @@
 #endif
     Loaded<H> bufA, bufB;
     issue_meta<H>(p, dir, ub, tile_of(0), tbase_of(0), tmr[0], off_l, 0, i16, kq, bufA);
-    issue_state<H>(hxb, ub, kq, bufA);
+    issue_state<H>(hxb, kq, bufA);
     auto item = [&](Loaded<H>& cur, Loaded<H>& nxt) -> int {
         int ns = s, ni = i + 1;
         if (sel(tT, ni) <= s) { ns = s + 1; ni = 0; }
@@ -313,11 +342,12 @@
 #ifdef OCRS_GRU_PROBE
         const uint64_t pt0 = __builtin_readcyclecounter();
 #endif
+        const f32x4 hp = own_piece<H>(cur, ub);
         float w[H / 4];
 #pragma unroll
         for (int j = 0; j < H / 16; j++) transpose4(cur.h[j], &w[4 * j]);
         if (have_next) issue_meta<H>(p, dir, ub, tile_of(ni), tbase_of(ni), sel(tmr, ni), off_l, ns, i16, kq, nxt);
-        if (early) issue_state<H>(hxb, ub, kq, nxt);
+        if (early) issue_state<H>(hxb, kq, nxt);
 #ifdef OCRS_GRU_PROBE
         asm volatile("" :: "v"(w[0]), "v"(w[H / 4 - 1]));
         const uint64_t pt1 = __builtin_readcyclecounter();
@@ -327,15 +357,15 @@
         asm volatile("" :: "v"(acc.r), "v"(acc.z), "v"(acc.n));
         const uint64_t pt2 = __builtin_readcyclecounter();
 #endif
-        const f32x4 hn = epilogue_store<H, FAST>(hxb, acc, cur.gr, cur.gz, cur.gn, cur.hp, cur.hx_off, cur.active, local);
+        const f32x4 hn = epilogue_store<H, FAST>(hxb, acc, cur.gr, cur.gz, cur.gn, hp, cur.hx_off, cur.active, local);
         store_local(yb, cur.active ? cur.out_off : 0xFFFFFFF0u, hn);
 #ifdef OCRS_GRU_PROBE
         const uint64_t pt3 = __builtin_readcyclecounter();
         pr_tr += pt1 - pt0; pr_mma += pt2 - pt1; pr_gate += pt3 - pt2; pr_items++;
 #endif
         if (!have_next) return 0;
-        if (!early) issue_state<H>(hxb, ub, kq, nxt);
-        if (!await_state<H>(p, hxb, ub, kq, nxt)) return -1;
+        if (!early) issue_state<H>(hxb, kq, nxt);
+        if (!await_state<H>(p, hxb, kq, nxt)) return -1;
 #ifdef OCRS_GRU_PROBE
         pr_wait += __builtin_readcyclecounter() - pt3;
 #endif
@@ -444,12 +474,11 @@
         for (int s = 0; s < T; s++) {
             L.active = tm > s;
             L.has_prev = L.active && s > 0;
-            L.hp = zero;
 #pragma unroll
             for (int j = 0; j < H / 16; j++) L.h[j] = zero;
             L.prev_off = L.has_prev ? (blk0 + s - 1u) * (H / 16) * 1024u + i16 * 64u : 0u;
-            issue_state<H>(hxb, ub, kq, L);
-            if (!await_state<H>(p, hxb, ub, kq, L)) *abort_w = 1;
+            issue_state<H>(hxb, kq, L);
+            if (!await_state<H>(p, hxb, kq, L)) *abort_w = 1;
             float w[H / 4];
 #pragma unroll
             for (int j = 0; j < H / 16; j++)
@@ -472,10 +501,11 @@
             const f32x4 zero = {0.0f, 0.0f, 0.0f, 0.0f};
             r_ = z_ = n_ = zero;
             if (a_) {
-                const float* g = p.gx + ((int64_t)dir * p.R + row) * 3 * H + ub * 16 + kq * 4;
+                const float* g = p.gx + ((int64_t)dir * p.R + row) * 3 * H + gru_gx_col(H, p.gx_blocked != 0, 0, ub * 16 + kq * 4);
+                const int gs = p.gx_blocked ? 16 : H;
                 r_ = *reinterpret_cast<const f32x4*>(g);
-                z_ = *reinterpret_cast<const f32x4*>(g + H);
-                n_ = *reinterpret_cast<const f32x4*>(g + 2 * H);
+                z_ = *reinterpret_cast<const f32x4*>(g + gs);
+                n_ = *reinterpret_cast<const f32x4*>(g + 2 * gs);
             }
         };
         fetch(0, gr, gz, gn, out_off, active);
@@ -648,7 +678,7 @@
 }
 
 bool gru_persistent(const float* gx, const float* wh, const float* bh, float* y, float* hx, const int32_t* d_Tm, const int32_t* d_off,
-                    const int32_t* h_Tm, int64_t R, int M, int Tmax, int H, uint32_t* d_sync, hipStream_t s) {
+                    const int32_t* h_Tm, int64_t R, int M, int Tmax, int H, bool gx_blocked, uint32_t* d_sync, hipStream_t s) {
     if (M <= 0) return true;
     if (!hx || !gru_persistent_supported(h_Tm, M, Tmax, R, H)) return false;
     const bool fast = option(OPT_NUMERICS) != 0;
@@ -663,6 +693,7 @@
     p.prio = 3;
     p.spin_limit = 1u << 21;
     p.allow_local = option(OPT_GRU_LOCAL) != 0;
+    p.gx_blocked = gx_blocked ? 1 : 0;
     const int UB = H / 16;
     if (option(OPT_GRU_GATES) && gru_gates_plan(M, Tmax, H, &p.ncl)) {
         for (int k = 0; k < p.ncl; k++) p.tbase[k] = base[k];
diff --git a/ocrs_amd/csrc/kernels_nn.hip b/ocrs_amd/csrc/kernels_nn.hip
--- a/ocrs_amd/csrc/kernels_nn.hip
+++ b/ocrs_amd/csrc/kernels_nn.hip
@@ -982,7 +982,7 @@
 
 __global__ void __launch_bounds__(256)
 gru_gates_kernel(const float* __restrict__ gx, const float* __restrict__ gh, float* __restrict__ h,
-                 float* __restrict__ y, int T, int N, int H, int step) {
+                 float* __restrict__ y, int T, int N, int H, int step, bool gxb) {
     const int dir = blockIdx.y;
     const int t = dir ? T - 1 - step : step;
     const int64_t total = (int64_t)N * H;
@@ -994,9 +994,9 @@
         const int64_t b = i / H;
         const float* gxr = gxp + b * 3 * H;
         const float* ghr = ghp + b * 3 * H;
-        float r = spec_sigmoidf(gxr[j] + ghr[j]);
-        float z = spec_sigmoidf(gxr[H + j] + ghr[H + j]);
-        float nn = spec_tanhf(fmaf(r, ghr[2 * H + j], gxr[2 * H + j]));
+        float r = spec_sigmoidf(gxr[gru_gx_col(H, gxb, 0, j)] + ghr[j]);
+        float z = spec_sigmoidf(gxr[gru_gx_col(H, gxb, 1, j)] + ghr[H + j]);
+        float nn = spec_tanhf(fmaf(r, ghr[2 * H + j], gxr[gru_gx_col(H, gxb, 2, j)]));
         float hprev = hp[i];
         float hn = fmaf(z, hprev - nn, nn);
         hp[i] = hn;
@@ -1004,11 +1004,11 @@
     }
 }
 
-void gru_gates(const float* gx, const float* gh, float* h, float* y, int T, int N, int H, int step, hipStream_t s) {
+void gru_gates(const float* gx, const float* gh, float* h, float* y, int T, int N, int H, int step, bool gx_blocked, hipStream_t s) {
     int64_t total = (int64_t)N * H;
     int grid = (int)((total + 255) / 256 < 4096 ? (total + 255) / 256 : 4096);
     if (grid < 1) grid = 1;
-    hipLaunchKernelGGL(gru_gates_kernel, dim3(grid, 2), dim3(256), 0, s, gx, gh, h, y, T, N, H, step);
+    hipLaunchKernelGGL(gru_gates_kernel, dim3(grid, 2), dim3(256), 0, s, gx, gh, h, y, T, N, H, step, gx_blocked && gru_gx_blockable(H));
 }
 
 constexpr int LSM_ROWS = 64;
@@ -1111,7 +1111,7 @@
 __global__ void __launch_bounds__(256)
 gru_gates_packed_kernel(const float* __restrict__ gx, const float* __restrict__ gh, float* __restrict__ h,
                         float* __restrict__ y, const int32_t* __restrict__ Tm, const int32_t* __restrict__ off,
-                        int64_t R, int Mcap, int active, int H, int step) {
+                        int64_t R, int Mcap, int active, int H, int step, bool gxb) {
     const int dir = blockIdx.y;
     const int64_t total = (int64_t)active * H;
     const float* gxd = gx + (int64_t)dir * R * 3 * H;
@@ -1124,9 +1124,9 @@
         const int64_t row = (int64_t)off[t] + m;
         const float* gxr = gxd + row * 3 * H;
         const float* ghr = ghd + (int64_t)m * 3 * H;
-        float r = spec_sigmoidf(gxr[j] + ghr[j]);
-        float z = spec_sigmoidf(gxr[H + j] + ghr[H + j]);
-        float nn = spec_tanhf(fmaf(r, ghr[2 * H + j], gxr[2 * H + j]));
+        float r = spec_sigmoidf(gxr[gru_gx_col(H, gxb, 0, j)] + ghr[j]);
+        float z = spec_sigmoidf(gxr[gru_gx_col(H, gxb, 1, j)] + ghr[H + j]);
+        float nn = spec_tanhf(fmaf(r, ghr[2 * H + j], gxr[gru_gx_col(H, gxb, 2, j)]));
         float hprev = hd[i];
         float hn = fmaf(z, hprev - nn, nn);
         hd[i] = hn;
@@ -1141,7 +1141,7 @@
 gru_step_fused_kernel(const float* __restrict__ gx, const float* __restrict__ wh, const float* __restrict__ bh,
                       const float* __restrict__ hT_in, float* __restrict__ hT_out, float* __restrict__ y,
                       const int32_t* __restrict__ Tm, const int32_t* __restrict__ off, int64_t R, int Mcap, int active,
-                      int step) {
+                      int step, bool gxb) {
     extern __shared__ __attribute__((aligned(16))) float lds_w[];
     const int dir = blockIdx.z;
     const int j0 = blockIdx.y * 16;
@@ -1179,9 +1179,9 @@
             const int t = dir ? Tm[m] - 1 - step : step;
             const int64_t row = (int64_t)off[t] + m;
             const float* g = gxd + row * 3 * H;
-            gxr_[r] = g[j];
-            gxz_[r] = g[H + j];
-            gxn_[r] = g[2 * H + j];
+            gxr_[r] = g[gru_gx_col(H, gxb, 0, j)];
+            gxz_[r] = g[gru_gx_col(H, gxb, 1, j)];
+            gxn_[r] = g[gru_gx_col(H, gxb, 2, j)];
             hprev_[r] = hin[(int64_t)j * Mcap + m];
             yrow[r] = row;
         }
@@ -1232,31 +1232,31 @@
 
 bool gru_step_fused(const float* gx, const float* wh, const float* bh, const float* hT_in, float* hT_out, float* y,
                     const int32_t* d_Tm, const int32_t* d_off, int64_t R, int Mcap, int active, int H, int step,
-                    hipStream_t s) {
+                    bool gx_blocked, hipStream_t s) {
     if (active <= 0) return true;
     dim3 grid((active + 63) / 64, H / 16, 2);
     size_t lds = (size_t)H * 48 * sizeof(float);
     if (H == 256)
         hipLaunchKernelGGL((gru_step_fused_kernel<256>), grid, dim3(256), lds, s, gx, wh, bh, hT_in, hT_out, y, d_Tm, d_off,
-                           R, Mcap, active, step);
+                           R, Mcap, active, step, gx_blocked);
     else if (H == 128)
         hipLaunchKernelGGL((gru_step_fused_kernel<128>), grid, dim3(256), lds, s, gx, wh, bh, hT_in, hT_out, y, d_Tm, d_off,
-                           R, Mcap, active, step);
+                           R, Mcap, active, step, gx_blocked);
     else if (H == 64)
         hipLaunchKernelGGL((gru_step_fused_kernel<64>), grid, dim3(256), lds, s, gx, wh, bh, hT_in, hT_out, y, d_Tm, d_off, R,
-                           Mcap, active, step);
+                           Mcap, active, step, gx_blocked);
     else
         return false;
     return true;
 }
 
 void gru_gates_packed(const float* gx, const float* gh, float* h, float* y, const int32_t* d_Tm, const int32_t* d_off,
-                      int64_t R, int Mcap, int active, int H, int step, hipStream_t s) {
+                      int64_t R, int Mcap, int active, int H, int step, bool gx_blocked, hipStream_t s) {
     int64_t total = (int64_t)active * H;
     if (total <= 0) return;
     int grid = (int)((total + 255) / 256 < 4096 ? (total + 255) / 256 : 4096);
     hipLaunchKernelGGL(gru_gates_packed_kernel, dim3(grid, 2), dim3(256), 0, s, gx, gh, h, y, d_Tm, d_off, R, Mcap, active,
-                       H, step);
+                       H, step, gx_blocked && gru_gx_blockable(H));
 }
 
 __global__ void __launch_bounds__(64)
diff --git a/ocrs_amd/csrc/model.cpp b/ocrs_amd/csrc/model.cpp
--- a/ocrs_amd/csrc/model.cpp
+++ b/ocrs_amd/csrc/model.cpp
@@ -137,6 +137,19 @@
                 }
                 pad16();
             }
+            if (gru_gx_blockable(f.hidden)) {
+                const int H3 = 3 * f.hidden;
+                for (int part = 0; part < 2; part++) {
+                    fixes.push_back({i, 4 + part, slab.size()});
+                    const int64_t rows = part == 0 ? f.cin : 1;
+                    for (int d = 0; d < 2; d++) {
+                        const float* src = blob + f.w[4 * d + part].off;
+                        for (int64_t r = 0; r < rows; r++)
+                            for (int c = 0; c < H3; c++) slab.push_back(src[r * H3 + gru_gx_to_natural(f.hidden, c)]);
+                    }
+                    pad16();
+                }
+            }
         }
         m->ops.push_back(op);
     }
@@ -182,7 +195,9 @@
         if (fx.which == 0) op.aux0 = p;
         else if (fx.which == 1) op.aux1 = p;
         else if (fx.which == 2) op.aux2 = p;
-        else op.aux3 = p;
+        else if (fx.which == 3) op.aux3 = p;
+        else if (fx.which == 4) op.aux0b = p;
+        else op.aux1b = p;
     }
     for (uint32_t i = 0; i < hd.n_ops; i++) {
         GraphOp& op = m->ops[i];
@@ -639,8 +654,9 @@
                 auto gh = get((size_t)2 * N * 3 * H);
                 auto hs = get((size_t)2 * N * H);
                 OCRS_HIP(hipMemsetAsync(hs.first, 0, (size_t)2 * N * H * sizeof(float), st));
+                const bool gxb = op.aux0b && option(OPT_GRU_GX_BLOCKED) != 0;
                 k::GemmDesc d{};
-                d.A = x; d.lda = I; d.B = op.aux0; d.ldb = 3 * H; d.bias = op.aux1; d.C = gx.first; d.ldc = 3 * H;
+                d.A = x; d.lda = I; d.B = gxb ? op.aux0b : op.aux0; d.ldb = 3 * H; d.bias = gxb ? op.aux1b : op.aux1; d.C = gx.first; d.ldc = 3 * H;
                 d.M = T * N; d.N = 3 * H; d.K = I; d.batch = 2;
                 d.strideA = 0; d.strideB = (int64_t)I * 3 * H; d.strideBias = 3 * H; d.strideC = (int64_t)T * N * 3 * H;
                 timed(KC_GEMM_GRU_INPUT, 2.0 * 2 * d.M * (double)d.N * d.K,
@@ -653,7 +669,7 @@
                     timed(KC_GEMM_GRU_HIDDEN, 2.0 * 2 * r.M * (double)r.N * r.K,
                           4.0 * 2 * ((double)r.M * r.K + (double)r.M * r.N + (double)r.K * r.N), [&] { k::gemm(r, st); });
                     timed(KC_GRU_GATES, 0, 4.0 * 2 * N * (double)H * 9,
-                          [&] { k::gru_gates(gx.first, gh.first, hs.first, y, T, N, H, step, st); });
+                          [&] { k::gru_gates(gx.first, gh.first, hs.first, y, T, N, H, step, gxb, st); });
                 }
                 free_local.emplace(gx.second, gx.first);
                 free_local.emplace(gh.second, gh.first);
@@ -1140,8 +1156,9 @@
             float* hxf = persistent && !split ? static_cast<float*>(hx_buf) : nullptr;
             if (split) OCRS_HIP(k::gru_split_prepare(hx, plan.h_Tm.data(), M, H, np, st));
             else if (persistent) OCRS_HIP(k::gru_persistent_prepare(hxf, plan.h_Tm.data(), M, H, st));
+            const bool gxb = op.aux0b && option(OPT_GRU_GX_BLOCKED) != 0 && np == 0 && !(range && range->gx_only && i == last);
             k::GemmDesc d{};
-            d.A = cur; d.lda = I; d.B = op.aux0; d.ldb = 3 * H; d.bias = op.aux1; d.C = gx; d.ldc = 3 * H;
+            d.A = cur; d.lda = I; d.B = gxb ? op.aux0b : op.aux0; d.ldb = 3 * H; d.bias = gxb ? op.aux1b : op.aux1; d.C = gx; d.ldc = 3 * H;
             d.M = (int)R; d.N = 3 * H; d.K = I; d.batch = 2;
             d.strideA = 0; d.strideB = (int64_t)I * 3 * H; d.strideBias = 3 * H; d.strideC = R * 3 * H;
             d.Bsplit = op.wsplit; d.strideBsplit = (int64_t)(3 * H / 128) * (I / 16) * 3 * 128 * 16;
@@ -1166,7 +1183,7 @@
                     OCRS_HIP(hipStreamWaitEvent(rs, ready, 0));
                     int ktok = timers ? timers->kbegin(KC_GEMM_GRU_HIDDEN, rs, fl, 4.0 * ((double)R * (2.0 * 3 * H + 2.0 * 2 * H) + 2.0 * 3 * H * H)) : -1;
                     ran_persistent = split ? k::gru_persistent_split(gx, op.aux2, op.aux3, y, hx, plan.d_Tm, plan.d_off, plan.h_Tm.data(), R, M, plan.Tmax, H, np, d_sync, rs)
-                                           : k::gru_persistent(gx, op.aux2, op.aux3, y, hxf, plan.d_Tm, plan.d_off, plan.h_Tm.data(), R, M, plan.Tmax, H, d_sync, rs);
+                                           : k::gru_persistent(gx, op.aux2, op.aux3, y, hxf, plan.d_Tm, plan.d_off, plan.h_Tm.data(), R, M, plan.Tmax, H, gxb, d_sync, rs);
                     if (ktok >= 0) timers->end(ktok, rs);
                     if (ran_persistent && plan.h_status && gru_layer < 8)
                         ws.download(plan.h_status + gru_layer, d_sync + k::gru_persistent_sync_words(M) - 1, sizeof(uint32_t), rs);
@@ -1187,7 +1204,7 @@
                     float* hout = (step & 1) ? hT0 : hT1;
                     timed(KC_GEMM_GRU_HIDDEN, 2.0 * 2 * act * 3.0 * H * H,
                           4.0 * 2 * ((double)act * H * 2 + (double)act * 3 * H + 3.0 * H * H + (double)act * H), [&] {
-                              if (!k::gru_step_fused(gx, op.aux2, op.aux3, hin, hout, y, plan.d_Tm, plan.d_off, R, Mcap, act, H, step, st))
+                              if (!k::gru_step_fused(gx, op.aux2, op.aux3, hin, hout, y, plan.d_Tm, plan.d_off, R, Mcap, act, H, step, gxb, st))
                                   fail(OCRS_ERR_RUN_FAILED, "model run failed: no fused GRU step kernel for hidden size %d", H);
                           });
                 }
@@ -1206,7 +1223,7 @@
                     timed(KC_GEMM_GRU_HIDDEN, 2.0 * 2 * act * (double)r.N * r.K,
                           4.0 * 2 * ((double)act * r.K + (double)act * r.N + (double)r.K * r.N), [&] { k::gemm(r, st); });
                     timed(KC_GRU_GATES, 0, 4.0 * 2 * act * (double)H * 9, [&] {
-                        k::gru_gates_packed(gx, gh, hs, y, plan.d_Tm, plan.d_off, R, M, act, H, step, st);
+                        k::gru_gates_packed(gx, gh, hs, y, plan.d_Tm, plan.d_off, R, M, act, H, step, gxb, st);
                     });
                 }
             }
diff --git a/ocrs_amd/csrc/model.hpp b/ocrs_amd/csrc/model.hpp
--- a/ocrs_amd/csrc/model.hpp
+++ b/ocrs_amd/csrc/model.hpp
@@ -23,6 +23,8 @@
     const float* aux1 = nullptr;
     const float* aux2 = nullptr;
     const float* aux3 = nullptr;
+    const float* aux0b = nullptr;
+    const float* aux1b = nullptr;
     const uint16_t* wsplit = nullptr;
     bool fused_into_prev = false;
     bool fuse_next_pw = false;
```
